# vLAR-group/OGC

Measured on AMD Instinct MI355X. Metric: point-clouds/sec (8192 pts) segnet fwd+bwd, higher is better.
Workload: dtype f32; 1 GPU; C4 KITTI-SF train_seg unsup: segnet_kitti fwd + OGC loss (dynamic+smooth+invariance) + bwd + Adam, 4 samples x 4 views x 8192 pts per GPU; n_point=8192, n_slot=10, parallelism=dp1, optimizer_stepped=True

## Files before the change

include/ogc_ops.h:

```cpp
#ifndef OGC_OPS_H
#define OGC_OPS_H

#ifdef __cplusplus
extern "C" {
#endif

typedef void *ogc_stream_t;
typedef unsigned short ogc_bf16_t;

enum {
    OGC_OK = 0,
    OGC_ERR_INVALID_ARG = -1,
    OGC_ERR_LAUNCH = -2,
    OGC_ERR_UNSUPPORTED = -3
};

#define OGC_VERSION 208
int ogc_version(void);
int ogc_distance_contracted(void);
int ogc_set_deterministic(int on);
int ogc_get_deterministic(void);
const char *ogc_last_error(void);

int ogc_furthest_point_sampling(int b, int n, int m, const float *xyz, float *temp,
// ... 150 lines not shown

int ogc_soft_carry(int b, int n1, int n2, int c, float temperature, const float *p1, const float *p2, const float *x,
                   float *out, ogc_stream_t stream);

#define OGC_SCAN_CROP_TILE 1024
#define OGC_SCAN_CROP_CAMERA_DOUBLES 36
int ogc_scan_crop_camera(int n, int stride, const float *scan, const double *cam, float clip_distance, float depth_thresh,
                         float *out_pc, int *keep_idx, int *count, ogc_stream_t stream);
int ogc_scan_crop_front(int n, int stride, const float *scan, float *out_pc, int *keep_idx, int *count, ogc_stream_t stream);
int ogc_scan_crop_tile(void);

#define OGC_BOX_SEGM_CHUNK 128
#define OGC_BOX_SEGM_BOX_DOUBLES 18
int ogc_box_segm(int n, int k, const float *pc, int sign_x, int sign_y, int sign_z, const double *boxes, const int *ids,
                 int *segm, int *semantic_segm, ogc_stream_t stream);
int ogc_box_segm_chunk(void);

int ogc_kittisf_unproject(int height, int width, const unsigned short *disp1, const unsigned short *disp2,
                          const unsigned short *flow, const unsigned short *inst, float fb, float f, float p02, float p03,
                          float p12, float p13, float p23, float depth_thresh, const int *select_semantics, int n_select,
                          float *pc1, float *pc2, int *segm, int *keep_idx, int *count, ogc_stream_t stream);

int ogc_png_unfilter(const unsigned char *in, unsigned char *out, int height, int row_bytes, int bpp);

int ogc_attention_fwd(int b, int lq, int lk, int h, int d, float scale, const float *q, int ldq, const float *k,
                      int ldk, const float *v, int ldv, float *out, float *prob, ogc_stream_t stream);
int ogc_attention_bwd(int b, int lq, int lk, int h, int d, float scale, const float *q, int ldq, const float *k,
                      int ldk, const float *v, int ldv, const float *out, const float *prob, const float *dout,
                      float *dq, int lddq, float *dk, int lddk, float *dv, int lddv, ogc_stream_t stream);

int ogc_small_linear_fwd(int rows, int n_in, int n_out, const float *x, const float *weight, const float *bias,
                         float *y, ogc_stream_t stream);
int ogc_small_linear_bwd(int rows, int n_in, int n_out, const float *x, const float *weight, const float *grad_y,
                         float *grad_x, float *grad_weight, float *grad_bias, ogc_stream_t stream);

int ogc_conv1x1_wgrad_moments(int b, int cin, int cout, int hw, int relu, const float *y_prev, const float *pa,
                              const float *pb, const float *grad_y, float *moments, ogc_stream_t stream);
int ogc_gn_moments_combine(int b, int cin, int cout, int hw, int groups, const float *moments, const float *w,
                           const float *pa, const float *pb, const float *mean, const float *rstd, const float *gamma,
                           float *grad_w, float *coef, float *grad_gamma, float *grad_beta, ogc_stream_t stream);
int ogc_conv1x1_dgrad_adjoint(int b, int cin, int cout, int hw, int relu, const float *w, const float *grad_y,
                              const float *y_prev, const float *pa, const float *pb, const float *coef, float *grad_prev,
                              ogc_stream_t stream);

int ogc_first_conv_stats(int b, int c1, int c0, int hw, int groups, const float *x0, const float *w1, double *stats,
                         ogc_stream_t stream);
int ogc_conv1x1_gemm_affine_first(int b, int M, int K, int hw, int relu, int groups, int c0, const float *w, const float *x0,
                                  const float *w1, const float *pa, const float *pb, float *out, double *stats,
                                  ogc_stream_t stream);
int ogc_conv1x1_wgrad_moments_first(int b, int cin, int cout, int hw, int relu, int c0, const float *x0, const float *w1,
                                    const float *pa, const float *pb, const float *grad_y, float *moments,
                                    ogc_stream_t stream);
int ogc_conv1x1_dgrad_adjoint_first(int b, int cin, int cout, int hw, int relu, int c0, const float *w, const float *grad_y,
                                    const float *x0, const float *w1, const float *pa, const float *pb, const float *coef,
                                    float *grad_w1, ogc_stream_t stream);

int ogc_group_norm_maxpool_bwd_sparse(int b, int c, int p, int s, int groups, int relu, const float *x,
                                      const float *x_at_argmax, const float *gamma, const float *mean, const float *rstd, const float *out, const int *argmax,
                                      const float *grad_out, float *coef2, float *inj, float *grad_gamma,
                                      float *grad_beta, double *ws, ogc_stream_t stream);
int ogc_conv1x1_wgrad_moments_pooled(int b, int cin, int cout, int hw, int relu, int nsample, const float *y_prev,
                                     const float *pa, const float *pb, const float *y, const float *coef2,
                                     const float *inj, float *moments, ogc_stream_t stream);
int ogc_conv1x1_dgrad_adjoint_pooled(int b, int cin, int cout, int hw, int relu, int nsample, const float *w, const float *y,
                                     const float *coef2, const float *inj, const float *y_prev, const float *pa,
                                     const float *pb, const float *coef, float *grad_prev, ogc_stream_t stream);

int ogc_live_steps(int b, int p, int nsample, const int *idx, int *live, int *n_live, ogc_stream_t stream);
int ogc_conv1x1_wgrad_moments_pooled_live(int b, int cin, int cout, int hw, int relu, int nsample, const float *y_prev,
                                          const float *pa, const float *pb, const float *y, const float *coef2,
                                          const float *inj, const int *live, const int *n_live, int live_cap, float *moments,
                                          ogc_stream_t stream);
int ogc_conv1x1_dgrad_adjoint_pooled_live(int b, int cin, int cout, int hw, int relu, int nsample, const float *w, const float *y,
                                          const float *coef2, const float *inj, const float *y_prev, const float *pa,
                                          const float *pb, const float *coef, const int *live, const int *n_live, int live_cap,
                                          float *grad_prev, ogc_stream_t stream);
int ogc_conv1x1_wgrad_moments_first_live(int b, int cin, int cout, int hw, int relu, int c0, int nsample, const float *x0,
                                         const float *w1, const float *pa, const float *pb, const float *grad_y,
                                         const int *live, const int *n_live, int live_cap, float *moments, ogc_stream_t stream);
int ogc_conv1x1_dgrad_adjoint_first_live(int b, int cin, int cout, int hw, int relu, int c0, int nsample, const float *w,
                                         const float *grad_y, const float *x0, const float *w1, const float *pa, const float *pb,
                                         const float *coef, const int *live, const int *n_live, int live_cap, float *grad_w1,
                                         ogc_stream_t stream);

int ogc_mlp_chain_pool_supported(int c0, int c1, int c2, int c3, int nsample);
int ogc_mlp_chain_pool(int b, int c0, int c1, int c2, int c3, int p, int nsample, const float *x, const float *wt1,
                       const float *b1, const float *wt2, const float *b2, const float *wt3, const float *b3, float *out,
                       ogc_stream_t stream);

int ogc_corr_layer_pool_supported(int cf, int c1, int c2, int c3, int nsample);
int ogc_corr_layer_pool(int b, int cf, int c1, int c2, int c3, int n1, int n2, int nsample, const float *pos1,
                        const float *pos2, const float *feat1, const float *feat2, const int *idx, const float *wt1,
                        const float *b1, const float *wt2, const float *b2, const float *wt3, const float *b3, float *out,
                        ogc_stream_t stream);

long long ogc_slot_masks_ws_floats(int b, int d, int n, int k);
int ogc_slot_masks_fwd(int b, int d, int n, int k, float temperature, const float *feats, const float *slots,
                       float *mask, ogc_stream_t stream);
int ogc_slot_masks_bwd(int b, int d, int n, int k, float temperature, const float *feats, const float *slots,
                       const float *mask, const float *grad_mask, float *grad_feats, float *grad_slots, float *ws,
                       ogc_stream_t stream);

int ogc_group_norm_stats_slots(void);
int ogc_group_norm_bwd_slots(void);
int ogc_group_norm_fwd(int b, int c, int hw, int groups, float eps, int relu, const float *x,
                       const float *gamma, const float *beta, float *y, float *mean, float *rstd,
                       double *ws, ogc_stream_t stream);
int ogc_group_norm_bwd(int b, int c, int hw, int groups, int relu, const float *x, const float *gamma,
                       const float *beta, const float *mean, const float *rstd, const float *grad_y,
                       float *grad_x, float *grad_gamma, float *grad_beta, double *ws, ogc_stream_t stream);

int ogc_group_norm_maxpool_fwd(int b, int c, int p, int s, int groups, float eps, int relu, const float *x,
                               const float *gamma, const float *beta, float *out, int *argmax, float *mean,
                               float *rstd, double *ws, ogc_stream_t stream);
int ogc_group_norm_maxpool_bwd(int b, int c, int p, int s, int groups, int relu, const float *x,
                               const float *gamma, const float *mean, const float *rstd, const float *out,
                               const int *argmax, const float *grad_out, float *grad_x, float *grad_gamma,
                               float *grad_beta, double *ws, ogc_stream_t stream);
int ogc_group_norm_maxpool_bwd_ext(int b, int c, int p, int s, int groups, int relu, const float *x,
                                   const float *x_at_argmax, const float *gamma, const float *mean, const float *rstd,
                                   const float *out, const int *argmax, const float *grad_out, float *grad_x,
                                   float *grad_gamma, float *grad_beta, double *ws, ogc_stream_t stream);

int ogc_batch_norm_fwd(int b, int c, int hw, float eps, int relu, int training, float momentum, const float *x,
                       const float *gamma, const float *beta, float *running_mean, float *running_var, float *y,
                       float *mean, float *rstd, double *ws, const double *stats, int slots, ogc_stream_t stream);
int ogc_batch_norm_bwd(int b, int c, int hw, int relu, int training, const float *x, const float *gamma,
                       const float *beta, const float *mean, const float *rstd, const float *grad_y, float *grad_x,
                       float *grad_gamma, float *grad_beta, double *ws, ogc_stream_t stream);
int ogc_batch_norm_maxpool_fwd(int b, int c, int p, int s, float eps, int relu, int training, float momentum,
                               const float *x, const float *gamma, const float *beta, float *running_mean,
                               float *running_var, float *out, int *argmax, float *mean, float *rstd, double *ws,
                               const double *stats, int slots, ogc_stream_t stream);
int ogc_batch_norm_maxpool_bwd(int b, int c, int p, int s, int relu, int training, const float *x, const float *gamma,
                               const float *mean, const float *rstd, const float *out, const int *argmax,
                               const float *grad_out, float *grad_x, float *grad_gamma, float *grad_beta, double *ws,
                               ogc_stream_t stream);

int ogc_conv1x1_wgrad(int b, int cin, int cout, int hw, const float *x, const float *dy, float *dw,
                      ogc_stream_t stream);

int ogc_conv1x1_gemm(int b, int M, int K, int hw, int transpose_a, const float *w, const float *in,
                     float *out, ogc_stream_t stream);

int ogc_conv1x1_gn_slots(void);
int ogc_conv1x1_gemm_stats_supported(int b, int M, int K, int hw, int affine);
int ogc_conv1x1_gemm_stream_supported(int b, int M, int K, int hw);
int ogc_conv1x1_gemm_any(int b, int M, int K, int hw, int transpose_a, const float *w, const float *in, float *out,
                         ogc_stream_t stream);

int ogc_set_matmul_precision(int bf16);
int ogc_conv1x1_gemm_gnstats(int b, int M, int K, int hw, int groups, const float *w, const float *in, float *out,
                             double *stats, ogc_stream_t stream);

int ogc_group_norm_coeffs(int b, int c, int hw, int groups, float eps, const float *x, const float *gamma,
                          const float *beta, const double *stats, int slots, double *ws, float *mean, float *rstd,
                          float *a, float *bb, ogc_stream_t stream);
int ogc_conv1x1_gemm_affine(int b, int M, int K, int hw, int relu, int groups, const float *w, const float *in,
                            const float *pa, const float *pb, float *out, double *stats, ogc_stream_t stream);
int ogc_conv1x1_wgrad_affine(int b, int cin, int cout, int hw, int relu, const float *x, const float *pa,
                             const float *pb, const float *dy, float *dw, ogc_stream_t stream);
int ogc_conv1x1_wgrad_affine_pooled(int b, int cin, int cout, int hw, int relu, int nsample, const float *x, const float *pa,
                                    const float *pb, const float *y, const float *coef2, const float *inj, float *dw,
                                    ogc_stream_t stream);
int ogc_conv1x1_dgrad_pooled(int b, int cin, int cout, int hw, int nsample, const float *w, const float *y, const float *coef2,
                             const float *inj, float *grad_z, ogc_stream_t stream);
// ... 87 lines not shown
```

ogc_amd/_lib.py:

```python
import ctypes
import os

_HERE = os.path.dirname(os.path.abspath(__file__))
FMAD = os.environ.get("OGC_FMAD", "0") == "1"
DETERMINISTIC = os.environ.get("OGC_DETERMINISTIC", "0") == "1"
LIB_PATH = os.path.join(_HERE, "csrc", "libogc_ops_fmad.so" if FMAD else "libogc_ops.so")

_vp = ctypes.c_void_p
_int = ctypes.c_int
_flt = ctypes.c_float
_dbl = ctypes.c_double
_ll = ctypes.c_longlong

SIGNATURES = {
    "ogc_set_deterministic": [_int],
    "ogc_group_linear_fwd_direct": [_int, _int, _int, _int, _int, _int, _int, _vp, _vp, _vp, _vp, _vp, _vp, _vp],
    "ogc_get_deterministic": [],
    "ogc_furthest_point_sampling": [_int, _int, _int, _vp, _vp, _vp, _vp],
    "ogc_furthest_point_sampling_chain": [_int, _int, _int, _vp, _vp, _vp, _vp, _vp, _vp],
    "ogc_gather_points": [_int, _int, _int, _int, _vp, _vp, _vp, _vp],
    "ogc_gather_points_grad": [_int, _int, _int, _int, _vp, _vp, _vp, _vp],
    "ogc_knn": [_int, _int, _int, _int, _vp, _vp, _vp, _vp, _vp],
    "ogc_three_nn": [_int, _int, _int, _vp, _vp, _vp, _vp, _vp],
    "ogc_three_interpolate": [_int, _int, _int, _int, _vp, _vp, _vp, _vp, _vp],
# ... 18 lines not shown
    "ogc_chamfer_terms": [_int, _int, _int, _int, _vp, _vp, _vp, _vp, _vp, _vp, _vp],
    "ogc_chamfer_terms_grad": [_int, _int, _int, _int, _vp, _vp, _vp, _vp, _vp, _vp, _vp, _vp],
    "ogc_gather_xyz_pair": [_int, _int, _int, _vp, _vp, _vp, _vp, _vp],
    "ogc_flow_advance": [_int, _int, _flt, _vp, _vp, _vp, _vp, _vp, _vp, _vp, _vp],
    "ogc_linear_cn": [_int, _int, _int, _int, _vp, _vp, _vp, _vp, _vp],
    "ogc_three_nn_weights": [_int, _int, _int, _vp, _vp, _vp],
    "ogc_soft_corr_flow": [_int, _int, _int, _int, _flt, _vp, _vp, _vp, _vp, _vp, _vp, _vp],
    "ogc_gru_reset": [_int, _int, _int, _int, _int, _vp, _ll, _vp, _vp, _vp],
    "ogc_gru_blend": [_int, _int, _int, _int, _vp, _ll, _vp, _ll, _vp, _ll, _vp, _vp],
    "ogc_zero_arena_begin": [_vp, _int, _vp],
    "ogc_zero_arena_end": [],
    "ogc_adam_max_tensors": [],
    "ogc_adam_chunk": [],
    "ogc_adam_step": [_int, _int, _vp, _vp, _vp, _vp, _vp, _dbl, _dbl, _dbl, _dbl, _dbl, _vp],
    "ogc_kabsch_rotation": [_int, _vp, _vp, _vp, _vp],
    "ogc_rigid_icp": [_int, _int, _vp, _vp, _vp, _int, _dbl, _vp, _vp, _vp, _vp],
    "ogc_ground_plane_fit": [_int, _int, _vp, _int, _int, _dbl, _dbl, _int, _vp, _vp, _vp, _vp],
    "ogc_seg_eval": [_int, _int, _int, _vp, _vp, _int, _vp, _vp, _vp, _vp, _vp, _vp, _vp, _vp, _vp, _vp, _vp],
    "ogc_seg_eval_ignore": [_int, _int, _int, _vp, _vp, _vp, _int, _vp, _vp, _vp, _vp, _vp, _vp, _vp, _vp, _vp, _vp, _vp, _vp],
    "ogc_flow_eval": [_int, _int, _vp, _vp, _dbl, _dbl, _vp, _vp, _vp],
    "ogc_lsap_maximize": [_int, _int, _vp, _vp, _vp],
    "ogc_sup_loss_ws_doubles": [_int, _int, _int],
    "ogc_sup_match_cost": [_int, _int, _int, _vp, _vp, _vp, _int, _dbl, _dbl, _vp, _vp, _vp, _vp],
    "ogc_sup_mask_loss_fwd": [_int, _int, _int, _vp, _vp, _vp, _vp, _int, _dbl, _dbl, _vp, _vp, _vp, _vp],
    "ogc_sup_mask_loss_bwd": [_int, _int, _int, _vp, _vp, _vp, _vp, _int, _dbl, _dbl, _vp, _dbl, _dbl, _vp, _vp, _vp],
    "ogc_rigid_moments": [_int, _int, _int, _vp, _vp, _vp, _vp, _vp, _vp, _vp],
    "ogc_rigid_translation": [_int, _vp, _vp, _vp, _vp, _vp],
    "ogc_rigid_blend": [_int, _int, _int, _int, _int, _vp, _vp, _vp, _vp, _vp, _vp, _vp, _vp],
    "ogc_mask_iou": [_int, _int, _int, _vp, _vp, _vp, _vp, _vp],
    "ogc_matched_distance": [_int, _int, _int, _int, _int, _vp, _vp, _vp, _vp, _vp, _vp, _vp, _vp, _vp],
    "ogc_soft_nn_target": [_int, _int, _int, _int, _flt, _vp, _vp, _vp, _vp, _vp, _vp],
    "ogc_soft_carry": [_int, _int, _int, _int, _flt, _vp, _vp, _vp, _vp, _vp],
    "ogc_scan_crop_camera": [_int, _int, _vp, _vp, _flt, _flt, _vp, _vp, _vp, _vp],
    "ogc_scan_crop_front": [_int, _int, _vp, _vp, _vp, _vp, _vp],
    "ogc_scan_crop_tile": [],
    "ogc_box_segm": [_int, _int, _vp, _int, _int, _int, _vp, _vp, _vp, _vp, _vp],
    "ogc_box_segm_chunk": [],
    "ogc_kittisf_unproject": [_int, _int, _vp, _vp, _vp, _vp, _flt, _flt, _flt, _flt, _flt, _flt, _flt, _flt, _vp, _int,
                              _vp, _vp, _vp, _vp, _vp, _vp],
    "ogc_png_unfilter": [_vp, _vp, _int, _int, _int],
    "ogc_group_concat": [_int, _int, _int, _int, _int, _vp, _vp, _vp, _vp, _vp, _vp],
    "ogc_group_linear_fwd": [_int, _int, _int, _int, _int, _int, _vp, _vp, _vp, _vp, _vp, _vp, _vp],
    "ogc_group_linear_bwd": [_int, _int, _int, _int, _int, _vp, _vp, _vp, _vp, _vp, _vp],
    "ogc_group_concat_grad": [_int, _int, _int, _int, _int, _vp, _vp, _vp, _vp],
    "ogc_neighbour_consistency_fwd": [_int, _int, _int, _int, _int, _vp, _vp, _vp, _vp],
    "ogc_reverse_neighbours": [_int, _int, _int, _vp, _vp, _vp, _vp, _vp, _vp],
    "ogc_neighbour_consistency_bwd": [_int, _int, _int, _int, _int, _vp, _vp, _vp, _vp, _vp, _vp, _vp, _vp],
    "ogc_sym_eigvals": [_int, _int, _vp, _vp, _vp],
    "ogc_group_norm_fwd": [_int, _int, _int, _int, _flt, _int, _vp, _vp, _vp, _vp, _vp, _vp, _vp, _vp],
    "ogc_group_norm_bwd": [_int, _int, _int, _int, _int, _vp, _vp, _vp, _vp, _vp, _vp, _vp, _vp, _vp, _vp, _vp],
    "ogc_group_norm_maxpool_fwd": [_int, _int, _int, _int, _int, _flt, _int, _vp, _vp, _vp, _vp, _vp, _vp, _vp, _vp, _vp],
    "ogc_conv1x1_gemm": [_int, _int, _int, _int, _int, _vp, _vp, _vp, _vp],
    "ogc_attention_fwd": [_int, _int, _int, _int, _int, _flt, _vp, _int, _vp, _int, _vp, _int, _vp, _vp, _vp],
    "ogc_attention_bwd": [_int, _int, _int, _int, _int, _flt, _vp, _int, _vp, _int, _vp, _int, _vp, _vp, _vp, _vp, _int,
                          _vp, _int, _vp, _int, _vp],
    "ogc_conv1x1_gemm_affine_pool": [_int, _int, _int, _int, _int, _int, _int, _vp, _vp, _vp, _vp, _vp, _vp, _vp, _vp, _vp,
                                     _vp],
    "ogc_group_norm_pool_extremes": [_int, _int, _int, _int, _int, _flt, _int, _vp, _vp, _vp, _vp, _vp, _vp, _vp, _vp, _vp,
                                     _int, _vp],
    "ogc_small_linear_fwd": [_int, _int, _int, _vp, _vp, _vp, _vp, _vp],
    "ogc_small_linear_bwd": [_int, _int, _int, _vp, _vp, _vp, _vp, _vp, _vp, _vp],
    "ogc_conv1x1_wgrad_moments": [_int, _int, _int, _int, _int, _vp, _vp, _vp, _vp, _vp, _vp],
    "ogc_gn_moments_combine": [_int, _int, _int, _int, _int, _vp, _vp, _vp, _vp, _vp, _vp, _vp, _vp, _vp, _vp, _vp, _vp],
    "ogc_conv1x1_dgrad_adjoint": [_int, _int, _int, _int, _int, _vp, _vp, _vp, _vp, _vp, _vp, _vp, _vp],
    "ogc_first_conv_stats": [_int, _int, _int, _int, _int, _vp, _vp, _vp, _vp],
    "ogc_conv1x1_gemm_affine_first": [_int, _int, _int, _int, _int, _int, _int, _vp, _vp, _vp, _vp, _vp, _vp, _vp, _vp],
    "ogc_conv1x1_wgrad_moments_first": [_int, _int, _int, _int, _int, _int, _vp, _vp, _vp, _vp, _vp, _vp, _vp],
    "ogc_conv1x1_dgrad_adjoint_first": [_int, _int, _int, _int, _int, _int, _vp, _vp, _vp, _vp, _vp, _vp, _vp, _vp, _vp],
    "ogc_group_norm_maxpool_bwd_sparse": [_int, _int, _int, _int, _int, _int, _vp, _vp, _vp, _vp, _vp, _vp, _vp, _vp, _vp, _vp,
                                          _vp, _vp, _vp, _vp],
    "ogc_group_norm_maxpool_bwd_ext": [_int, _int, _int, _int, _int, _int, _vp, _vp, _vp, _vp, _vp, _vp, _vp, _vp, _vp, _vp,
                                       _vp, _vp, _vp],
    "ogc_conv1x1_wgrad_moments_pooled": [_int, _int, _int, _int, _int, _int, _vp, _vp, _vp, _vp, _vp, _vp, _vp, _vp],
    "ogc_conv1x1_dgrad_adjoint_pooled": [_int, _int, _int, _int, _int, _int, _vp, _vp, _vp, _vp, _vp, _vp, _vp, _vp, _vp, _vp],
    "ogc_live_steps": [_int, _int, _int, _vp, _vp, _vp, _vp],
    "ogc_conv1x1_wgrad_moments_pooled_live": [_int, _int, _int, _int, _int, _int, _vp, _vp, _vp, _vp, _vp, _vp, _vp, _vp, _int, _vp,
                                              _vp],
    "ogc_conv1x1_dgrad_adjoint_pooled_live": [_int, _int, _int, _int, _int, _int, _vp, _vp, _vp, _vp, _vp, _vp, _vp, _vp, _vp, _vp,
                                              _int, _vp, _vp],
    "ogc_conv1x1_wgrad_moments_first_live": [_int, _int, _int, _int, _int, _int, _int, _vp, _vp, _vp, _vp, _vp, _vp, _vp, _int, _vp,
                                             _vp],
    "ogc_conv1x1_dgrad_adjoint_first_live": [_int, _int, _int, _int, _int, _int, _int, _vp, _vp, _vp, _vp, _vp, _vp, _vp, _vp, _vp,
                                             _int, _vp, _vp],
    "ogc_mlp_chain_pool_supported": [_int, _int, _int, _int, _int],
    "ogc_mlp_chain_pool":[_int, _int, _int, _int, _int, _int, _int, _vp, _vp, _vp, _vp, _vp, _vp, _vp, _vp, _vp],
    "ogc_corr_layer_pool_supported": [_int, _int, _int, _int, _int],
    "ogc_corr_layer_pool": [_int, _int, _int, _int, _int, _int, _int, _int, _vp, _vp, _vp, _vp, _vp, _vp, _vp, _vp, _vp, _vp,
                            _vp, _vp, _vp],
    "ogc_slot_masks_ws_floats": [_int, _int, _int, _int],
    "ogc_slot_masks_fwd": [_int, _int, _int, _int, _flt, _vp, _vp, _vp, _vp],
    "ogc_slot_masks_bwd": [_int, _int, _int, _int, _flt, _vp, _vp, _vp, _vp, _vp, _vp, _vp, _vp],
    "ogc_conv1x1_gn_slots": [],
    "ogc_conv1x1_gemm_stats_supported": [_int, _int, _int, _int, _int],
    "ogc_conv1x1_gemm_stream_supported": [_int, _int, _int, _int],
    "ogc_conv1x1_gemm_any": [_int, _int, _int, _int, _int, _vp, _vp, _vp, _vp],
    "ogc_set_matmul_precision": [_int],
    "ogc_group_norm_stats_slots": [],
    "ogc_group_norm_bwd_slots": [],
    "ogc_group_norm_coeffs": [_int, _int, _int, _int, _flt, _vp, _vp, _vp, _vp, _int, _vp, _vp, _vp, _vp, _vp, _vp],
    "ogc_conv1x1_gemm_affine": [_int, _int, _int, _int, _int, _int, _vp, _vp, _vp, _vp, _vp, _vp, _vp],
    "ogc_conv1x1_wgrad_affine": [_int, _int, _int, _int, _int, _vp, _vp, _vp, _vp, _vp, _vp],
    "ogc_conv1x1_wgrad_affine_pooled": [_int, _int, _int, _int, _int, _int, _vp, _vp, _vp, _vp, _vp, _vp, _vp, _vp],
    "ogc_conv1x1_dgrad_pooled": [_int, _int, _int, _int, _int, _vp, _vp, _vp, _vp, _vp, _vp],
    "ogc_batch_norm_fwd": [_int, _int, _int, _flt, _int, _int, _flt, _vp, _vp, _vp, _vp, _vp, _vp, _vp, _vp, _vp, _vp,
                           _int, _vp],
    "ogc_batch_norm_bwd": [_int, _int, _int, _int, _int, _vp, _vp, _vp, _vp, _vp, _vp, _vp, _vp, _vp, _vp, _vp],
    "ogc_batch_norm_maxpool_fwd": [_int, _int, _int, _int, _flt, _int, _int, _flt, _vp, _vp, _vp, _vp, _vp, _vp, _vp,
                                   _vp, _vp, _vp, _vp, _int, _vp],
    "ogc_batch_norm_maxpool_bwd": [_int, _int, _int, _int, _int, _int, _vp, _vp, _vp, _vp, _vp, _vp, _vp, _vp, _vp,
                                   _vp, _vp, _vp],
    "ogc_conv1x1_gemm_gnstats": [_int, _int, _int, _int, _int, _vp, _vp, _vp, _vp, _vp],
    "ogc_group_norm_fwd_stats": [_int, _int, _int, _int, _flt, _int, _vp, _vp, _vp, _vp, _vp, _vp, _vp, _int, _vp],
    "ogc_group_norm_maxpool_fwd_stats": [_int, _int, _int, _int, _int, _flt, _int, _vp, _vp, _vp, _vp, _vp, _vp, _vp,
                                         _vp, _int, _vp],
    "ogc_conv1x1_wgrad": [_int, _int, _int, _int, _vp, _vp, _vp, _vp],
    "ogc_group_norm_maxpool_bwd": [_int, _int, _int, _int, _int, _int, _vp, _vp, _vp, _vp, _vp, _vp, _vp, _vp, _vp, _vp,
                                   _vp, _vp],
}

for _n in ("ogc_group_linear_fwd", "ogc_group_points_grad_rev", "ogc_conv1x1_gemm", "ogc_conv1x1_gemm_affine",
           "ogc_conv1x1_gemm_affine_pool", "ogc_conv1x1_wgrad_affine", "ogc_conv1x1_wgrad_affine_pooled",
           "ogc_conv1x1_dgrad_pooled", "ogc_conv1x1_wgrad_moments", "ogc_conv1x1_wgrad_moments_pooled",
           "ogc_conv1x1_dgrad_adjoint", "ogc_conv1x1_dgrad_adjoint_pooled", "ogc_group_norm_bwd",
           "ogc_group_norm_maxpool_bwd_sparse", "ogc_group_points_grad_rev_dwx"):
    SIGNATURES[_n + "_h"] = SIGNATURES[_n]
SIGNATURES["ogc_group_linear_fwd_direct_h"] = SIGNATURES["ogc_group_linear_fwd_direct"]
SIGNATURES["ogc_conv1x1_wgrad_xf_h"] = SIGNATURES["ogc_conv1x1_wgrad"]
SIGNATURES["ogc_group_linear_fwd_pt_h"] = SIGNATURES["ogc_group_linear_fwd"]

HEADER_VERSION = 208
_lib = None
_fns = {}


class OgcOpsError(RuntimeError):
    pass


def load():
    global _lib
    if _lib is None:
        if not os.path.exists(LIB_PATH):
            raise OgcOpsError(
                "libogc_ops.so not found at %s — build it with `python ogc_amd/csrc/build.py` "
                "(there is no CPU fallback)" % LIB_PATH)
        L = ctypes.CDLL(LIB_PATH)
        for name, argtypes in SIGNATURES.items():
            fn = getattr(L, name)
            fn.argtypes = argtypes
            fn.restype = _int
        L.ogc_version.restype = _int
        if L.ogc_version() != HEADER_VERSION:
            raise OgcOpsError("libogc_ops.so at %s is version %d, this package binds version %d of include/ogc_ops.h — rebuild it "
                              "with `python ogc_amd/csrc/build.py --force`" % (LIB_PATH, L.ogc_version(), HEADER_VERSION))
        L.ogc_distance_contracted.restype = _int
        if bool(L.ogc_distance_contracted()) != FMAD:
            raise OgcOpsError("%s evaluates distances %s, OGC_FMAD asked for the other form" %
                              (LIB_PATH, "contracted (fma)" if L.ogc_distance_contracted() else "un-contracted"))
        L.ogc_slot_masks_ws_floats.restype = ctypes.c_longlong
        L.ogc_cell_grid_bytes.restype = ctypes.c_longlong
        L.ogc_sup_loss_ws_doubles.restype = ctypes.c_longlong
        L.ogc_last_error.restype = ctypes.c_char_p
        L.ogc_set_deterministic(1 if DETERMINISTIC else 0)
        _lib = L
    return _lib

# ... 61 lines not shown
```

ogc_amd/csrc/build.py:

```python
import os
import subprocess
import sys
from concurrent.futures import ThreadPoolExecutor

HERE = os.path.dirname(os.path.abspath(__file__))
SOURCES = ["api.hip", "det.hip", "knn.hip", "ball_query.hip", "fps.hip", "gather_group.hip", "interpolate.hip", "kabsch.hip", "rigid_icp.hip", "ground_plane.hip", "seg_eval.hip", "flow_eval.hip", "sup_loss.hip", "small_solvers.hip", "neighbour_loss.hip", "soft_nn.hip", "soft_carry.hip", "scan_prepare.hip", "kittisf_prepare.hip", "seg_loss.hip", "group_norm.hip", "batch_norm.hip", "grid.hip", "grid_ball_query.hip", "grid_knn.hip", "conv1x1.hip", "conv1x1_h.hip", "conv1x1_wgrad.hip", "attention.hip", "slot_masks.hip", "small_linear.hip", "loss_glue.hip", "mlp_chain.hip", "gn_fused_bwd.hip", "adam.hip", "gemm_chunk.hip", "chamfer.hip", "flow_step.hip"]
HEADERS = ["ogc_common.h", "grid.h", "grid_dev.h", "conv_stage.h", "conv1x1_shared.h", "act_io.h", "norm_dev.h", "conv1x1_epilogue.h", "first_conv.h", "wgrad_tile_body.inc", "wgrad_shared_body.inc", "svd3.h", "png_unfilter.h", os.path.join("..", "..", "include", "ogc_ops.h")]
LIB = os.path.join(HERE, "libogc_ops.so")
FMAD_SOURCES = ["knn.hip", "ball_query.hip", "fps.hip", "grid.hip", "grid_ball_query.hip", "grid_knn.hip"]
LIB_FMAD = os.path.join(HERE, "libogc_ops_fmad.so")
HIPCC = os.environ.get("HIPCC", "/opt/rocm/bin/hipcc")
FLAGS = [
    "--offload-arch=gfx950", "-O3", "-std=c++17", "-fPIC",
    "-ffp-contract=off",
    "-munsafe-fp-atomics",
    "-mllvm", "-amdgpu-mfma-vgpr-form=1",
    "-Wall", "-Wno-unused-function",
]


def _newer(target, deps):
    if not os.path.exists(target):
        return True
    t = os.path.getmtime(target)
    return any(os.path.getmtime(d) > t for d in deps)


def build(force=False, verbose=False):
    hdrs = [os.path.join(HERE, h) for h in HEADERS] + [os.path.abspath(__file__)]
    objs, objs_fmad, jobs = [], [], []
    for s in SOURCES:
        src = os.path.join(HERE, s)
        obj = os.path.join(HERE, s.replace(".hip", ".o"))
        objs.append(obj)
        if force or _newer(obj, [src] + hdrs):
            jobs.append([HIPCC] + FLAGS + ["-c", src, "-o", obj])
        if s in FMAD_SOURCES:
            obj_f = os.path.join(HERE, s.replace(".hip", ".fmad.o"))
            objs_fmad.append(obj_f)
            if force or _newer(obj_f, [src] + hdrs):
                jobs.append([HIPCC] + FLAGS + ["-DOGC_FMAD=1", "-c", src, "-o", obj_f])
        else:
            objs_fmad.append(obj)

    def run(cmd):
        if verbose:
            print(" ".join(cmd), flush=True)
        subprocess.check_call(cmd)

    with ThreadPoolExecutor(max_workers=min(8, max(1, len(jobs)))) as ex:
        list(ex.map(run, jobs))
    if force or jobs or _newer(LIB, objs):
        run([HIPCC, "--offload-arch=gfx950", "-shared", "-fPIC", "-o", LIB] + objs)
    if force or jobs or _newer(LIB_FMAD, objs_fmad):
        run([HIPCC, "--offload-arch=gfx950", "-shared", "-fPIC", "-o", LIB_FMAD] + objs_fmad)
    return LIB


if __name__ == "__main__":
    print(build(force="--force" in sys.argv, verbose="--verbose" in sys.argv))
```

ogc_amd/csrc/conv1x1.hip:

```cpp
#include "conv1x1_shared.h"
#include "act_io.h"
#include "conv1x1_epilogue.h"
#include "first_conv.h"

int ogc_g_matmul_bf16 = 0;


namespace {


template <bool TRANSPOSE_A, int KQ, bool STATS, bool PRO, bool BF, bool POOL = false, typename IT = float, typename OT = float,
          int FIRST = 0>
__global__ __launch_bounds__(WG_WAVES *OGC_WAVE) void conv1x1_gemm_kernel(int M, int K, int hw, int groups,
                                                                          const float *__restrict__ w,
                                                                          const IT *__restrict__ in,
                                                                          OT *__restrict__ out,
                                                                          double *__restrict__ stats,
                                                                          const float *__restrict__ pa,
                                                                          const float *__restrict__ pb, int pro_relu,
                                                                          PoolOut pool = PoolOut(), FirstIn first = FirstIn()) {
    extern __shared__ __attribute__((aligned(16))) float a_lds[];
    __shared__ __attribute__((aligned(16))) float s_w1[FIRST ? FC_MAX_ROWS * FC_MAX_C0 : 4];
    __shared__ double s_stats[STATS ? 64 : 1];
    __shared__ __attribute__((aligned(16))) float s_sign[POOL ? 64 : 4];
    const int lane = threadIdx.x & 63, wave = threadIdx.x >> 6;
    const int j = lane & 15, kk = lane >> 4;
    const int b = blockIdx.y;
    const int p0 = (blockIdx.x * WG_WAVES + wave) * 64;
    const int Kq = (K + 3) >> 2, a_ld = ogc_a_ld(Kq);
    const bool live = p0 < hw;
    const IT *inb = in + (size_t)b * K * hw;
    OT *outb = out + (size_t)b * M * hw;
    if (STATS && threadIdx.x < 2 * groups) s_stats[threadIdx.x] = 0.0;

    float4 xin[KQ];
    if constexpr (FIRST > 0) {
        static_assert(KQ * 4 <= FC_MAX_ROWS && sizeof(IT) == 4 && !TRANSPOSE_A, "first-layer form: fp32, at most 64 rows of W1");
        ogc_first_stage_w1<WG_WAVES * OGC_WAVE>(s_w1, first.w1, K, first.c0);
        float4 x0v[FIRST];
        ogc_first_load_raw<FIRST>(x0v, first.x0 + (size_t)b * first.c0 * hw + (live ? p0 + 4 * j : 0), first.c0, hw);
        ogc_first_mask<FIRST>(x0v, first.c0, live);
        __syncthreads();
#pragma unroll
        for (int q = 0; q < KQ; ++q) {
            float w1r[FIRST];
            ogc_first_w1_row<FIRST>(w1r, s_w1, q * 4 + kk);
            xin[q] = ogc_first_row<FIRST>(x0v, w1r);
        }
    } else {
#pragma unroll
    for (int q = 0; q < KQ; ++q) {
        const int row = q * 4 + kk;
        xin[q] = (live && q < Kq && row < K) ? ogc_ld4(inb + (size_t)row * hw + p0 + 4 * j) : make_float4(0.f, 0.f, 0.f, 0.f);
    }
    }
    if (PRO) {
        constexpr int CH = 8;
#pragma unroll
        for (int q0 = 0; q0 < KQ; q0 += CH) {
            float ca[CH], cb[CH];
#pragma unroll
            for (int u = 0; u < CH; ++u) {
                const int q = q0 + u, row = q * 4 + kk;
                const bool have = q < KQ && live && q < Kq && row < K;
                ca[u] = have ? pa[(size_t)b * K + row] : 0.f;
                cb[u] = have ? pb[(size_t)b * K + row] : 0.f;
            }
#pragma unroll
            for (int u = 0; u < CH; ++u) {
                const int q = q0 + u;
                if (q < KQ) {
                    float4 v = xin[q];
                    v.x = fmaf(ca[u], v.x, cb[u]); v.y = fmaf(ca[u], v.y, cb[u]);
                    v.z = fmaf(ca[u], v.z, cb[u]); v.w = fmaf(ca[u], v.w, cb[u]);
                    if (pro_relu) { v.x = fmaxf(v.x, 0.f); v.y = fmaxf(v.y, 0.f); v.z = fmaxf(v.z, 0.f); v.w = fmaxf(v.w, 0.f); }
                    xin[q] = v;
                }
            }
        }
    }
    constexpr int GQ = (KQ + 3) / 4;
    v4s xb[BF ? GQ : 1][4];
    if constexpr (BF) {
#pragma unroll
        for (int g = 0; g < GQ; ++g) {
            float4 r[4];
#pragma unroll
            for (int i = 0; i < 4; ++i) r[i] = 4 * g + i < KQ ? xin[4 * g + i] : make_float4(0.f, 0.f, 0.f, 0.f);
            xb[g][0] = ogc_pack_bf16(r[0].x, r[1].x, r[2].x, r[3].x);
            xb[g][1] = ogc_pack_bf16(r[0].y, r[1].y, r[2].y, r[3].y);
            xb[g][2] = ogc_pack_bf16(r[0].z, r[1].z, r[2].z, r[3].z);
            xb[g][3] = ogc_pack_bf16(r[0].w, r[1].w, r[2].w, r[3].w);
        }
    }
    const int cpg = STATS ? M / groups : 1;
    for (int m0 = 0; m0 < M; m0 += 64) {
        __syncthreads();
        if constexpr (BF) {
            v4s *a_bf = reinterpret_cast<v4s *>(a_lds);
            const int Gq = (Kq + 3) >> 2;
            for (int t = threadIdx.x; t < Gq * 256; t += WG_WAVES * OGC_WAVE) {
                const int kr = t & 3, mi = (t >> 2) & 63, g = t >> 8;
                const int m = m0 + mi;
                float v[4];
#pragma unroll
                for (int i = 0; i < 4; ++i) {
                    const int k = 4 * (4 * g + i) + kr;
                    v[i] = (m < M && k < K) ? (TRANSPOSE_A ? w[(size_t)k * M + m] : w[(size_t)m * K + k]) : 0.f;
                }
                a_bf[t] = ogc_pack_bf16(v[0], v[1], v[2], v[3]);
            }
        } else {
        ogc_stage_weight_tile<TRANSPOSE_A, WG_WAVES>(a_lds, w, m0, M, K, Kq);
        }
        if constexpr (POOL) {
            if (threadIdx.x < 64) s_sign[threadIdx.x] = (m0 + (int)threadIdx.x < M && pool.sign[m0 + threadIdx.x] < 0.f) ? -1.f : 1.f;
        }
        __syncthreads();
        const int nblk = min(4, (M - m0 + 15) >> 4);
        v4f acc[4][4];
#pragma unroll
        for (int a = 0; a < 4; ++a)
#pragma unroll
            for (int c = 0; c < 4; ++c) acc[a][c] = (v4f){0.f, 0.f, 0.f, 0.f};
        if constexpr (BF) {
            const v4s *a_bf = reinterpret_cast<const v4s *>(a_lds);
#pragma unroll
            for (int g = 0; g + 1 < GQ; g += 2) {
                if (4 * (g + 1) < Kq) {
                    v4s av0[4], av1[4];
#pragma unroll
                    for (int a = 0; a < 4; ++a) {
                        av0[a] = a_bf[(g * 64 + a * 16 + j) * 4 + kk];
                        av1[a] = a_bf[((g + 1) * 64 + a * 16 + j) * 4 + kk];
                    }
#pragma unroll
                    for (int a = 0; a < 4; ++a) {
                        if (a < nblk) {
#pragma unroll
                            for (int c = 0; c < 4; ++c)
                                acc[a][c] = ogc_mfma_bf16_k32(av0[a], av1[a], xb[g][c], xb[g + 1][c], acc[a][c]);
                        }
                    }
                } else if (4 * g < Kq) {
                    v4s av[4];
#pragma unroll
                    for (int a = 0; a < 4; ++a) av[a] = a_bf[(g * 64 + a * 16 + j) * 4 + kk];
#pragma unroll
                    for (int a = 0; a < 4; ++a) {
                        if (a < nblk) {
#pragma unroll
                            for (int c = 0; c < 4; ++c)
                                acc[a][c] = __builtin_amdgcn_mfma_f32_16x16x16bf16_1k(av[a], xb[g][c], acc[a][c], 0, 0, 0);
                        }
                    }
                }
            }
            if constexpr (GQ % 2 == 1) {
                constexpr int g = GQ - 1;
                if (4 * g < Kq) {
                    v4s av[4];
#pragma unroll
                    for (int a = 0; a < 4; ++a) av[a] = a_bf[(g * 64 + a * 16 + j) * 4 + kk];
#pragma unroll
                    for (int a = 0; a < 4; ++a) {
                        if (a < nblk) {
#pragma unroll
                            for (int c = 0; c < 4; ++c)
                                acc[a][c] = __builtin_amdgcn_mfma_f32_16x16x16bf16_1k(av[a], xb[g][c], acc[a][c], 0, 0, 0);
                        }
                    }
                }
            }
        } else {
#pragma unroll
        for (int q = 0; q < KQ; ++q) {
            if (q < Kq) {
                float av[4];
#pragma unroll
                for (int a = 0; a < 4; ++a) av[a] = a_lds[(a * 16 + j) * a_ld + q * 4 + kk];
#pragma unroll
                for (int a = 0; a < 4; ++a) {
                    if (a < nblk) {
                        acc[a][0] = __builtin_amdgcn_mfma_f32_16x16x4f32(av[a], xin[q].x, acc[a][0], 0, 0, 0);
                        acc[a][1] = __builtin_amdgcn_mfma_f32_16x16x4f32(av[a], xin[q].y, acc[a][1], 0, 0, 0);
                        acc[a][2] = __builtin_amdgcn_mfma_f32_16x16x4f32(av[a], xin[q].z, acc[a][2], 0, 0, 0);
                        acc[a][3] = __builtin_amdgcn_mfma_f32_16x16x4f32(av[a], xin[q].w, acc[a][3], 0, 0, 0);
                    }
                }
            }
        }
        }
        if (live) {
            if constexpr (sizeof(OT) == 2 && (STATS || POOL)) {
#pragma unroll
                for (int a = 0; a < 4; ++a)
#pragma unroll
                    for (int c = 0; c < 4; ++c)
#pragma unroll
                        for (int r = 0; r < 4; ++r) acc[a][c][r] = ogc_as_stored<OT>(acc[a][c][r]);
            }
#pragma unroll
            for (int a = 0; a < 4; ++a)
#pragma unroll
                for (int r = 0; r < 4; ++r) {
                    const int m = m0 + a * 16 + kk * 4 + r;
                    if (m < M) {
                        const float4 o = make_float4(acc[a][0][r], acc[a][1][r], acc[a][2][r], acc[a][3][r]);
                        ogc_st4(outb + (size_t)m * hw + p0 + 4 * j, o);
                    }
                }
            if constexpr (POOL) {
                const int centres = hw / pool.s;
                const int centre = (p0 + 4 * j) / pool.s;
                const size_t o0 = ((size_t)b * M + m0 + kk * 4) * centres + centre;
                if (pool.s == 64) ogc_pool_extremes_epilogue<16>(acc, nblk, s_sign, j, kk, m0, M, centres, 64, pool.yext + o0, pool.aext + o0);
                else if (pool.s == 32) ogc_pool_extremes_epilogue<8>(acc, nblk, s_sign, j, kk, m0, M, centres, 32, pool.yext + o0, pool.aext + o0);
                else ogc_pool_extremes_epilogue<4>(acc, nblk, s_sign, j, kk, m0, M, centres, 16, pool.yext + o0, pool.aext + o0);
            }
            if (STATS) {
#pragma unroll
                for (int a = 0; a < 4; ++a) {
                    if (a < nblk) {
                        float sm = 0.f, sq = 0.f;
#pragma unroll
                        for (int r = 0; r < 4; ++r)
#pragma unroll
                            for (int c = 0; c < 4; ++c) {
                                const float v = acc[a][c][r];
                                sm += v;
                                sq += v * v;
                            }
                        sm += ogc_dpp_f32<0xB1>(sm); sq += ogc_dpp_f32<0xB1>(sq);
                        sm += ogc_dpp_f32<0x4E>(sm); sq += ogc_dpp_f32<0x4E>(sq);
                        sm += ogc_dpp_f32<0x141>(sm); sq += ogc_dpp_f32<0x141>(sq);
                        sm += ogc_dpp_f32<0x140>(sm); sq += ogc_dpp_f32<0x140>(sq);
                        const int m = m0 + a * 16 + kk * 4;
                        if (j == 0 && m < M) {
                            const int g = m / cpg;
                            atomicAdd(&s_stats[2 * g], (double)sm);
                            atomicAdd(&s_stats[2 * g + 1], (double)sq);
                        }
                    }
                }
            }
        }
    }
    if (STATS) {
        __syncthreads();
        if (threadIdx.x < 2 * groups) {
            const int slot = blockIdx.x % GN_SLOTS;
            double *dst = stats + ((size_t)slot * gridDim.y + b) * 2 * groups;
            atomicAdd(dst + threadIdx.x, s_stats[threadIdx.x]);
        }
    }
}

template <int KQ, bool PRO, bool EXACT, bool STATS = false, bool POOL = false, bool DUAL = false, bool TRANS = false>
__global__ __launch_bounds__(WG_WAVES *OGC_WAVE, DUAL ? 2 : 1) void conv1x1_gemm_stream_kernel(int M, int K, int hw, int ntiles,
                                                                                 const float *__restrict__ w,
                                                                                 const float *__restrict__ in,
                                                                                 float *__restrict__ out,
                                                                                 const float *__restrict__ pa,
                                                                                 const float *__restrict__ pb, int pro_relu,
                                                                                 int groups = 1, int nbatch = 1,
                                                                                 double *__restrict__ stats = nullptr,
                                                                                 PoolOut pool = PoolOut()) {
    extern __shared__ __attribute__((aligned(16))) float a_lds[];
    const int lane = threadIdx.x & 63, wave = __builtin_amdgcn_readfirstlane(threadIdx.x >> 6);
    const int j = lane & 15, kk = lane >> 4;
    const int Kq = (K + 3) >> 2, Mt = (M + 63) >> 6, a_ld = ogc_a_ld(Kq);
    const int tiles_per_img = hw >> 6;
    for (int mt = 0; mt < Mt; ++mt)
        ogc_stage_weight_tile<TRANS, WG_WAVES>(a_lds + (size_t)mt * 64 * a_ld, w, mt * 64, M, K, Kq);
    float *sgn_all = a_lds + (size_t)Mt * 64 * a_ld + (PRO ? WG_WAVES * 2 * FW_KQ_MAX * 4 : 0) + WG_WAVES * 4 * 16 * 2 * 2;
    if constexpr (POOL) {
        for (int t = threadIdx.x; t < Mt * 64; t += WG_WAVES * OGC_WAVE) sgn_all[t] = (t < M && pool.sign[t] < 0.f) ? -1.f : 1.f;
    }
    __syncthreads();
    const int nw = gridDim.x * WG_WAVES;
    const unsigned off_main = (unsigned)(kk * hw + 4 * j);
    const unsigned off_last = (unsigned)(min(kk, K - 1 - (Kq - 1) * 4) * hw + 4 * j);
    auto load_tile = [&](int t, float4(&x)[KQ]) {
        t = min(t, ntiles - 1);
        const int b = t / tiles_per_img, p0 = (t - b * tiles_per_img) * 64;
        const float *inb = in + (size_t)b * K * hw + p0;
#pragma unroll
        for (int q = 0; q < KQ; ++q)
            if (EXACT || q < Kq) {
                const float *rowq = inb + (size_t)(q * 4) * hw;
                x[q] = *reinterpret_cast<const float4 *>(rowq + ((EXACT ? q == KQ - 1 : q == Kq - 1) ? off_last : off_main));
            }
    };
    float *cw = a_lds + (size_t)Mt * 64 * a_ld + wave * (2 * KQ * 4);
    int coef_b = -1;
    double *sacc = reinterpret_cast<double *>(a_lds + (size_t)Mt * 64 * a_ld + (PRO ? WG_WAVES * 2 * FW_KQ_MAX * 4 : 0)) +
                   wave * (4 * 16 * 2);
    int stat_b = -1;
    auto flush_stats = [&]() {
        if constexpr (STATS) {
            if (stat_b >= 0) {
                const int cpg = M / groups;
                double *dst = stats + ((size_t)(blockIdx.x % GN_SLOTS) * nbatch + stat_b) * 2 * groups;
                if (lane < Mt * 16) {
                    const int m = (lane >> 4) * 64 + ((lane >> 2) & 3) * 16 + (lane & 3) * 4;
                    if (m < M) {
                        unsafeAtomicAdd(dst + 2 * (m / cpg), sacc[2 * lane]);
                        unsafeAtomicAdd(dst + 2 * (m / cpg) + 1, sacc[2 * lane + 1]);
                    }
                }
            }
            if (lane < 64) { sacc[2 * lane] = 0.0; sacc[2 * lane + 1] = 0.0; }
            __builtin_amdgcn_wave_barrier();
        }
    };
    auto compute_store = [&](int t, float4(&x)[KQ]) {
        const int b = t / tiles_per_img, p0 = (t - b * tiles_per_img) * 64;
        if constexpr (STATS) {
            if (b != stat_b) { flush_stats(); stat_b = b; }
// ... 412 lines not shown
        for (int a = 0; a < 4; ++a) {
            if (a < nblk) {
                float sm = 0.f, sq = 0.f;
#pragma unroll
                for (int r = 0; r < 4; ++r) {
                    float w[CP];
                    ogc_first_w1_row<CP>(w, s_w1, a * 16 + kk * 4 + r);
                    const float4 v = ogc_first_row<CP>(x, w);
                    sm += v.x; sq += v.x * v.x;
                    sm += v.y; sq += v.y * v.y;
                    sm += v.z; sq += v.z * v.z;
                    sm += v.w; sq += v.w * v.w;
                }
                sm += ogc_dpp_f32<0xB1>(sm); sq += ogc_dpp_f32<0xB1>(sq);
                sm += ogc_dpp_f32<0x4E>(sm); sq += ogc_dpp_f32<0x4E>(sq);
                sm += ogc_dpp_f32<0x141>(sm); sq += ogc_dpp_f32<0x141>(sq);
                sm += ogc_dpp_f32<0x140>(sm); sq += ogc_dpp_f32<0x140>(sq);
                dsm[a] += (double)sm;
                dsq[a] += (double)sq;
            }
        }
    }
    const int cpg = c1 / groups;
#pragma unroll
    for (int a = 0; a < 4; ++a) {
        const int m = a * 16 + kk * 4;
        if (j == 0 && m < c1) {
            atomicAdd(&s_stats[2 * (m / cpg)], dsm[a]);
            atomicAdd(&s_stats[2 * (m / cpg) + 1], dsq[a]);
        }
    }
    __syncthreads();
    if (threadIdx.x < 2 * groups) {
        double *dst = stats + ((size_t)(blockIdx.x % GN_SLOTS) * gridDim.y + b) * 2 * groups;
        atomicAdd(dst + threadIdx.x, s_stats[threadIdx.x]);
    }
}

int first_check(const char *name, int b, int c1, int c0, int hw, const float *x0, const float *w1) {
    OGC_REQUIRE(b >= 0 && c1 >= 1 && c0 >= 1 && hw >= 1, "%s: bad shape", name);
    OGC_REQUIRE(x0 && w1, "%s: null pointer", name);
    if (c0 > FC_MAX_C0 || c1 > FC_MAX_ROWS || (hw & 63) != 0 || ((uintptr_t)x0 & 15) != 0) {
        ogc_set_error("%s: needs c0 <= %d, c1 <= %d, hw %% 64 == 0 and a 16-byte aligned x0 (c0=%d, c1=%d, hw=%d)", name, FC_MAX_C0,
                      FC_MAX_ROWS, c0, c1, hw);
        return OGC_ERR_UNSUPPORTED;
    }
    OGC_REQUIRE((long long)FC_MAX_ROWS * hw < (1ll << 31) && b <= 32768, "%s: one sample exceeds 32-bit indexing", name);
    return OGC_OK;
}

}

int ogc_first_check(const char *name, int b, int c1, int c0, int hw, const float *x0, const float *w1) {
    return first_check(name, b, c1, c0, hw, x0, w1);
}

extern "C" int ogc_first_conv_stats(int b, int c1, int c0, int hw, int groups, const float *x0, const float *w1, double *stats,
                                    ogc_stream_t stream) {
    const int rc = first_check("ogc_first_conv_stats", b, c1, c0, hw, x0, w1);
    if (rc != OGC_OK) return rc;
    OGC_REQUIRE(stats, "ogc_first_conv_stats: null pointer");
    if (groups < 1 || groups > 32 || c1 % groups != 0 || (c1 / groups) % 4 != 0) {
        ogc_set_error("ogc_first_conv_stats: needs 1 <= groups <= 32 and (c1 / groups) %% 4 == 0 (c1=%d, groups=%d)", c1, groups);
        return OGC_ERR_UNSUPPORTED;
    }
    if (b == 0) return OGC_OK;
    hipStream_t s = (hipStream_t)stream;
    if (ogc_zero_async(stats, sizeof(double) * 2 * GN_SLOTS * (size_t)b * groups, s) != hipSuccess) {
        ogc_set_error("ogc_first_conv_stats: memset failed");
        return OGC_ERR_LAUNCH;
    }
    const int tiles = ogc_divup(hw, 64 * WG_WAVES);
    int run = ogc_divup((long long)tiles * b, 2048);
    if (run > 8) run = 8;
    dim3 grid(ogc_divup(tiles, run), b), block(WG_WAVES * OGC_WAVE);
    const int cp = ogc_first_cp(c0);
    if (cp == 3) hipLaunchKernelGGL(first_conv_stats_kernel<3>, grid, block, 0, s, c1, c0, hw, groups, run, x0, w1, stats);
    else if (cp == 6) hipLaunchKernelGGL(first_conv_stats_kernel<6>, grid, block, 0, s, c1, c0, hw, groups, run, x0, w1, stats);
    else hipLaunchKernelGGL(first_conv_stats_kernel<8>, grid, block, 0, s, c1, c0, hw, groups, run, x0, w1, stats);
    OGC_CHECK_LAUNCH("ogc_first_conv_stats");
    return OGC_OK;
}

extern "C" int ogc_conv1x1_gemm_affine_first(int b, int M, int K, int hw, int relu, int groups, int c0, const float *w,
                                             const float *x0, const float *w1, const float *pa, const float *pb, float *out,
                                             double *stats, ogc_stream_t stream) {
    const char *name = "ogc_conv1x1_gemm_affine_first";
    int rc = first_check(name, b, K, c0, hw, x0, w1);
    if (rc != OGC_OK) return rc;
    OGC_REQUIRE(M >= 1 && w && pa && pb && out && stats, "%s: bad shape or null pointer", name);
    if (groups < 1 || groups > 32 || M % groups != 0 || (M / groups) % 4 != 0 || ((uintptr_t)out & 15) != 0 || g_matmul_bf16) {
        ogc_set_error("%s: needs fp32 operands, 1 <= groups <= 32, (M / groups) %% 4 == 0 and a 16-byte aligned output (M=%d, "
                      "groups=%d)", name, M, groups);
        return OGC_ERR_UNSUPPORTED;
    }
    OGC_REQUIRE((long long)M * hw < (1ll << 31) && b <= 65535, "%s: one sample exceeds 32-bit indexing", name);
    if (b == 0) return OGC_OK;
    hipStream_t s = (hipStream_t)stream;
    if (ogc_zero_async(stats, sizeof(double) * 2 * GN_SLOTS * (size_t)b * groups, s) != hipSuccess) {
        ogc_set_error("%s: memset failed", name);
        return OGC_ERR_LAUNCH;
    }
    const int Kq = (K + 3) / 4, cp = ogc_first_cp(c0);
    const size_t lds = (size_t)64 * ogc_a_ld(Kq) * sizeof(float);
    dim3 grid(ogc_divup(hw, 64 * WG_WAVES), b);
    FirstIn first;
    first.x0 = x0; first.w1 = w1; first.c0 = c0;
#define OGC_GEMM_FIRST(KQV, CPV)                                                                                           \
    hipLaunchKernelGGL((conv1x1_gemm_kernel<false, KQV, true, true, false, false, float, float, CPV>), grid,               \
                       dim3(WG_WAVES * OGC_WAVE), lds, s, M, K, hw, groups, w, (const float *)nullptr, out, stats, pa, pb, relu, \
                       PoolOut(), first)
    if (Kq <= 8) {
        if (cp == 3) OGC_GEMM_FIRST(8, 3); else if (cp == 6) OGC_GEMM_FIRST(8, 6); else OGC_GEMM_FIRST(8, 8);
    } else {
        if (cp == 3) OGC_GEMM_FIRST(16, 3); else if (cp == 6) OGC_GEMM_FIRST(16, 6); else OGC_GEMM_FIRST(16, 8);
    }
#undef OGC_GEMM_FIRST
    OGC_CHECK_LAUNCH(name);
    return OGC_OK;
}
```

ogc_amd/csrc/conv1x1_epilogue.h:

```cpp
#pragma once
#include "conv1x1_shared.h"

namespace {

constexpr int FW_KQ_MAX = 40;
constexpr int GN_SLOTS = 16;

template <int CTRL>
__device__ __forceinline__ float ogc_max_dpp_f32(float x) {
    float r;
    if constexpr (CTRL == 0xB1)
        asm("s_nop 1\n\tv_max_f32_dpp %0, %1, %1 quad_perm:[1,0,3,2] row_mask:0xf bank_mask:0xf" : "=v"(r) : "v"(x));
    else if constexpr (CTRL == 0x4E)
        asm("s_nop 1\n\tv_max_f32_dpp %0, %1, %1 quad_perm:[2,3,0,1] row_mask:0xf bank_mask:0xf" : "=v"(r) : "v"(x));
    else if constexpr (CTRL == 0x141)
        asm("s_nop 1\n\tv_max_f32_dpp %0, %1, %1 row_half_mirror row_mask:0xf bank_mask:0xf" : "=v"(r) : "v"(x));
    else
        asm("s_nop 1\n\tv_max_f32_dpp %0, %1, %1 row_mirror row_mask:0xf bank_mask:0xf" : "=v"(r) : "v"(x));
    return r;
}
__device__ __forceinline__ float ogc_max3_f32(float a, float b, float c) {
    float r;
    asm("v_max3_f32 %0, %1, %2, %3" : "=v"(r) : "v"(a), "v"(b), "v"(c));
    return r;
}
__device__ __forceinline__ float ogc_max2_f32(float a, float b) {
    float r;
    asm("v_max_f32 %0, %1, %2" : "=v"(r) : "v"(a), "v"(b));
    return r;
}

struct PoolOut {
    float *yext;
    int *aext;
    const float *sign;
    int s;
};

template <int SEG, typename ACC>
__device__ __forceinline__ void ogc_pool_extremes_epilogue(const ACC (&acc)[4][4], int nblk, const float *sgn, int j, int kk,
                                                           int m0, int M, int centres, int pool_s, float *ye, int *ae) {
    const bool writer = (j & (SEG - 1)) == 0;
#pragma unroll
    for (int a = 0; a < 4; ++a) {
        if (a < nblk) {
            const float4 sg4 = *reinterpret_cast<const float4 *>(sgn + a * 16 + kk * 4);
            const float sga[4] = {sg4.x, sg4.y, sg4.z, sg4.w};
#pragma unroll
            for (int r = 0; r < 4; ++r) {
                const int m = m0 + a * 16 + kk * 4 + r;
                const float sg = sga[r];
                const float v0 = sg * acc[a][0][r], v1 = sg * acc[a][1][r];
                const float v2 = sg * acc[a][2][r], v3 = sg * acc[a][3][r];
                float hi = ogc_max3_f32(v0, v1, ogc_max2_f32(v2, v3));
                hi = ogc_max_dpp_f32<0xB1>(hi);
                hi = ogc_max_dpp_f32<0x4E>(hi);
                if (SEG >= 8) hi = ogc_max_dpp_f32<0x141>(hi);
                if (SEG >= 16) hi = ogc_max_dpp_f32<0x140>(hi);
                unsigned idx = v3 == hi ? 4u * j + 3u : 64u;
                idx = v2 == hi ? 4u * j + 2u : idx;
                idx = v1 == hi ? 4u * j + 1u : idx;
                idx = v0 == hi ? 4u * j : idx;
                idx = min(idx, ogc_dpp_u32<0xB1>(idx));
                idx = min(idx, ogc_dpp_u32<0x4E>(idx));
                if (SEG >= 8) idx = min(idx, ogc_dpp_u32<0x141>(idx));
                if (SEG >= 16) idx = min(idx, ogc_dpp_u32<0x140>(idx));
                if (writer && m < M) {
                    const int o = (a * 16 + r) * centres;
                    ye[o] = sg * hi;
                    ae[o] = (int)(idx & (unsigned)(pool_s - 1));
                }
            }
        }
    }
}

template <auto KERNEL, typename... ARGS>
bool ogc_persistent_launch(size_t lds, int lds_cap, int per_cu, long long ntiles, hipStream_t s, ARGS... args) {
    static bool raised = false;
    if (!raised) {
        if (hipFuncSetAttribute(reinterpret_cast<const void *>(KERNEL), hipFuncAttributeMaxDynamicSharedMemorySize, lds_cap) != hipSuccess) {
            (void)hipGetLastError();
            return false;
        }
        raised = true;
    }
    long long wgs = 256ll * per_cu;
    if (wgs > ntiles / WG_WAVES) wgs = ntiles / WG_WAVES;
    hipLaunchKernelGGL(KERNEL, dim3((unsigned)wgs), dim3(WG_WAVES * OGC_WAVE), lds, s, args...);
    return true;
}

}
```

ogc_amd/csrc/gn_fused_bwd.hip:

```cpp
#include "conv1x1_shared.h"
#include "act_io.h"
#include "first_conv.h"

namespace {

constexpr int LIVE_SHIFT = 28;
constexpr int LIVE_MASK = (1 << LIVE_SHIFT) - 1;
struct LiveIn {
    const int *steps = nullptr;
    const int *n = nullptr;
    int cap = 0;
};

constexpr int LIVE_MAX_P = 32768;
__global__ __launch_bounds__(1024) void live_steps_kernel(int p, int s, const int *__restrict__ idx, int *__restrict__ steps,
                                                          int *__restrict__ n_live) {
    __shared__ int part[1024];
    __shared__ unsigned char cnt[LIVE_MAX_P];
    const int t = threadIdx.x, b = blockIdx.x, T = s >> 4;
    const int lane = t & 63, wave = t >> 6;
    const int *ib = idx + (size_t)b * p * s;
    int *out = steps + (size_t)b * p * T;
    const int row0 = lane & ~(s - 1);
    const unsigned long long row_mask = (s == 64 ? ~0ull : (1ull << s) - 1ull) << row0;
    const int total = p * s;
    for (int e0 = wave * 64; e0 < total; e0 += 1024) {
        const bool in = e0 + lane < total;
        const int v = in ? ib[e0 + lane] : 0;
        const int first = __shfl(v, row0);
        const unsigned long long differs = __builtin_amdgcn_ballot_w64(in && v != first) & row_mask;
        const int hi = differs ? 63 - __clzll(differs) - row0 : 0;
        if (in && lane == row0) cnt[(e0 + lane) / s] = (unsigned char)(min((hi + 1) >> 4, T - 1) + 1);
    }
    __syncthreads();
    const int per = (p + 1023) / 1024;
    const int c0 = min(t * per, p), c1 = min(c0 + per, p);
    int sum = 0;
    for (int c = c0; c < c1; ++c) sum += cnt[c];
    part[t] = sum;
    __syncthreads();
    for (int off = 1; off < 1024; off <<= 1) {
        const int v = t >= off ? part[t - off] : 0;
        __syncthreads();
        part[t] += v;
        __syncthreads();
    }
    int at = t > 0 ? part[t - 1] : 0;
    for (int c = c0; c < c1; ++c) {
        const int sl = cnt[c] - 1;
        for (int st = 0; st <= sl; ++st) out[at++] = (c * T + st) | (st == sl ? (T - 1 - sl) << LIVE_SHIFT : 0);
    }
    if (t == 1023) n_live[b] = part[1023];
}

template <int COB, int CIB, bool POOLED, typename AT = float, int FIRST = 0, bool LIST = false>
__global__ __launch_bounds__(WG_WAVES *OGC_WAVE) void wgrad_moments_kernel(int cin, int cout, int hw, int chunks,
                                                                           int steps_per_wave, int relu,
                                                                           const AT *__restrict__ x,
                                                                           const AT *__restrict__ dy,
                                                                           const float *__restrict__ aff_a,
                                                                           const float *__restrict__ aff_b,
                                                                           const float2 *__restrict__ coef2,
                                                                           const float2 *__restrict__ inj,
                                                                           int s_shift,
                                                                           float *__restrict__ hm,
                                                                           FirstIn first = FirstIn(), LiveIn ls = LiveIn()) {
    constexpr int XN = FIRST ? FIRST : CIB;
    __shared__ float red[WG_WAVES][COB * CIB * 256];
    const int lane = threadIdx.x & 63, wave = __builtin_amdgcn_readfirstlane(threadIdx.x >> 6);
    const int i = lane & 15, k = lane >> 4;
    const int img = blockIdx.x / chunks, chunk = blockIdx.x - img * chunks;
    const int co0 = blockIdx.y * (16 * COB), ci0 = blockIdx.z * (16 * CIB);
    int steps_per_img = hw >> 4;
    const int *lv_ = nullptr;
    if constexpr (LIST) {
        steps_per_img = min(ls.n[img], ls.cap);
        lv_ = ls.steps + (size_t)img * ls.cap;
        const int waves = chunks * WG_WAVES;
        steps_per_wave = ((steps_per_img + waves - 1) / waves + 1) & ~1;
        if (chunk * WG_WAVES * steps_per_wave >= steps_per_img) return;
    }
    const int first_step = (chunk * WG_WAVES + wave) * steps_per_wave;
    const int mine = max(0, min(steps_per_wave, steps_per_img - first_step));

    v4f acc1[COB][CIB], acc2[COB][CIB];
#pragma unroll
    for (int a = 0; a < COB; ++a)
#pragma unroll
        for (int c = 0; c < CIB; ++c) {
            acc1[a][c] = (v4f){0.f, 0.f, 0.f, 0.f};
            acc2[a][c] = (v4f){0.f, 0.f, 0.f, 0.f};
        }
    int yrow[COB], xrow[XN], jrow[COB];
    float ca[CIB], cb[CIB], pc2[COB], pc3[COB];
    float w1r[FIRST ? CIB : 1][FIRST ? FIRST : 1];
    const int centres = hw >> s_shift, smask = (1 << s_shift) - 1;
#pragma unroll
    for (int a = 0; a < COB; ++a) {
        const int row = min(co0 + a * 16 + i, cout - 1);
        yrow[a] = row * hw;
        if (POOLED) {
            const float2 cc = coef2[(size_t)img * cout + row];
            pc2[a] = cc.x;
            pc3[a] = cc.y;
            jrow[a] = row * centres;
        }
    }
    const float2 *jb_ = POOLED ? inj + (size_t)img * cout * centres : nullptr;
#pragma unroll
    for (int c = 0; c < CIB; ++c) {
        const int ch = min(ci0 + c * 16 + i, cin - 1);
        if constexpr (FIRST == 0) xrow[c] = ch * hw;
        ca[c] = aff_a[(size_t)img * cin + ch];
        cb[c] = aff_b[(size_t)img * cin + ch];
        if constexpr (FIRST > 0) {
#pragma unroll
            for (int e = 0; e < FIRST; ++e) w1r[c][e] = e < first.c0 ? first.w1[ch * first.c0 + min(e, first.c0 - 1)] : 0.f;
        }
    }
    if constexpr (FIRST > 0) {
#pragma unroll
        for (int e = 0; e < FIRST; ++e) xrow[e] = min(e, first.c0 - 1) * hw;
    }
    const AT *yb_ = dy + (size_t)img * cout * hw + 4 * k;
    const AT *xb_ = FIRST ? reinterpret_cast<const AT *>(first.x0) + (size_t)img * first.c0 * hw + 4 * k
                          : x + (size_t)img * cin * hw + 4 * k;
    int cur = min(first_step, steps_per_img - 1);
    const int stop = min(first_step + mine, steps_per_img) - 1;
    int ent = LIST ? lv_[cur] : 0;
    auto load = [&](float4(&yv)[COB], float4(&xv)[XN], float2(&jv)[COB], int &jpos, int &went) {
        const int pb = LIST ? min(ent & LIVE_MASK, (hw >> 4) - 1) * 16 : cur * 16;
        if constexpr (LIST) went = ent;
#pragma unroll
        for (int a = 0; a < COB; ++a) yv[a] = ogc_ld4(yb_ + yrow[a] + pb);
#pragma unroll
// ... 496 lines not shown
                    for (int g = 0; g + 1 < GQ; g += 2) {
                        if (4 * (g + 1) < Kq) {
                            const v4s av0 = a_bf[(g * 64 + a * 16 + j) * 4 + kk], av1 = a_bf[((g + 1) * 64 + a * 16 + j) * 4 + kk];
#pragma unroll
                            for (int c = 0; c < 4; ++c) acc[c] = ogc_mfma_bf16_k32(av0, av1, xb[g][c], xb[g + 1][c], acc[c]);
                        } else if (4 * g < Kq) {
                            const v4s av = a_bf[(g * 64 + a * 16 + j) * 4 + kk];
#pragma unroll
                            for (int c = 0; c < 4; ++c) acc[c] = __builtin_amdgcn_mfma_f32_16x16x16bf16_1k(av, xb[g][c], acc[c], 0, 0, 0);
                        }
                    }
                    if constexpr (GQ % 2 == 1) {
                        constexpr int g = GQ - 1;
                        if (4 * g < Kq) {
                            const v4s av = a_bf[(g * 64 + a * 16 + j) * 4 + kk];
#pragma unroll
                            for (int c = 0; c < 4; ++c) acc[c] = __builtin_amdgcn_mfma_f32_16x16x16bf16_1k(av, xb[g][c], acc[c], 0, 0, 0);
                        }
                    }
                } else {
#pragma unroll
                for (int q = 0; q < KQ; ++q) {
                    if (q < Kq) {
                        const float av = a_lds[(a * 16 + j) * a_ld + q * 4 + kk];
                        acc[0] = __builtin_amdgcn_mfma_f32_16x16x4f32(av, xin[q].x, acc[0], 0, 0, 0);
                        acc[1] = __builtin_amdgcn_mfma_f32_16x16x4f32(av, xin[q].y, acc[1], 0, 0, 0);
                        acc[2] = __builtin_amdgcn_mfma_f32_16x16x4f32(av, xin[q].z, acc[2], 0, 0, 0);
                        acc[3] = __builtin_amdgcn_mfma_f32_16x16x4f32(av, xin[q].w, acc[3], 0, 0, 0);
                    }
                }
                }
                if (live) {
#pragma unroll
                    for (int r = 0; r < 4; ++r) {
                        const int mi = a * 16 + kk * 4 + r, m = m0 + mi;
                        if (m < M) {
                            const float fa = cf[mi * 5], fb = cf[mi * 5 + 1], al = cf[mi * 5 + 2], c2 = cf[mi * 5 + 3], c3 = cf[mi * 5 + 4];
                            const float4 y = yv[r];
                            float4 g = make_float4(acc[0][r], acc[1][r], acc[2][r], acc[3][r]);
                            if (relu) {
                                g.x = fmaf(fa, y.x, fb) > 0.f ? g.x : 0.f; g.y = fmaf(fa, y.y, fb) > 0.f ? g.y : 0.f;
                                g.z = fmaf(fa, y.z, fb) > 0.f ? g.z : 0.f; g.w = fmaf(fa, y.w, fb) > 0.f ? g.w : 0.f;
                            }
                            float4 o;
                            o.x = fmaf(al, g.x, fmaf(c2, y.x, c3)); o.y = fmaf(al, g.y, fmaf(c2, y.y, c3));
                            o.z = fmaf(al, g.z, fmaf(c2, y.z, c3)); o.w = fmaf(al, g.w, fmaf(c2, y.w, c3));
                            if constexpr (FIRST > 0) {
                                float mine = 0.f;
                                if constexpr (LIST) o.w *= wl;
#pragma unroll
                                for (int c = 0; c < FIRST; ++c) {
                                    float d = fmaf(o.w, x0v[c].w, fmaf(o.z, x0v[c].z, fmaf(o.y, x0v[c].y, o.x * x0v[c].x)));
                                    d += ogc_dpp_f32<0xB1>(d);
                                    d += ogc_dpp_f32<0x4E>(d);
                                    d += ogc_dpp_f32<0x141>(d);
                                    d += ogc_dpp_f32<0x140>(d);
                                    mine = j == c ? d : mine;
                                }
                                if (j < first.c0) atomicAdd(&s_dw[m * FC_MAX_C0 + j], mine);
                            } else {
                                if (mine_ok) ogc_st4(outb + (size_t)m * hw + pos, o);
                            }
                        }
                    }
                }
            }
        }
    }
    }
    if constexpr (FIRST > 0) {
        __syncthreads();
        for (int t = threadIdx.x; t < M * first.c0; t += WG_WAVES * OGC_WAVE) {
            const float v = s_dw[(t / first.c0) * FC_MAX_C0 + t % first.c0];
            if (v != 0.0f) unsafeAtomicAdd(first.dw1 + t, v);
        }
    }
}

}

namespace {
int nsample_shift(int nsample) { return nsample == 16 ? 4 : nsample == 32 ? 5 : nsample == 64 ? 6 : -1; }

int live_check(const char *name, const int *live, const int *n_live, int live_cap, int hw, int nsample, LiveIn &ls) {
    OGC_REQUIRE(live && n_live, "%s: null live-step list", name);
    if (nsample != 32 && nsample != 64) {
        ogc_set_error("%s: the list form needs nsample 32 or 64 (nsample=%d)", name, nsample);
        return OGC_ERR_UNSUPPORTED;
    }
    OGC_REQUIRE(hw >= 16 && hw % nsample == 0 && (hw >> 4) <= LIVE_MASK && live_cap >= (hw >> 4),
                "%s: the live-step list holds %d entries per sample, hw=%d needs room for %d", name, live_cap, hw, hw >> 4);
    ls.steps = live; ls.n = n_live; ls.cap = live_cap;
    return OGC_OK;
}

template <typename AT>
int wgrad_moments_impl(const char *name, int b, int cin, int cout, int hw, int relu, const AT *y_prev, const float *pa,
                       const float *pb, const AT *grad_y, const float *coef2, const float *inj, int s_shift,
                       float *moments, ogc_stream_t stream, LiveIn ls = LiveIn()) {
    OGC_REQUIRE(b >= 0 && cin >= 1 && cout >= 1 && hw >= 1, "%s: bad shape", name);
    OGC_REQUIRE(y_prev && pa && pb && grad_y && moments, "%s: null pointer", name);
    if ((hw & (sizeof(AT) == 2 ? 31 : 15)) != 0 || (((uintptr_t)y_prev | (uintptr_t)grad_y) & 15) != 0) {
        ogc_set_error("%s: hw=%d must be a multiple of 16 (32 for 16-bit tensors) and the tensors 16-byte aligned", name, hw);
        return OGC_ERR_UNSUPPORTED;
    }
    if (sizeof(AT) == 2 && !ogc_g_matmul_bf16) {
        ogc_set_error("%s: 16-bit activations need ogc_set_matmul_precision(1)", name);
        return OGC_ERR_UNSUPPORTED;
    }
    OGC_REQUIRE((long long)cin * hw < (1ll << 31) && (long long)cout * hw < (1ll << 31) && b <= 32768,
                "%s: one sample exceeds 32-bit indexing", name);
    hipStream_t s = (hipStream_t)stream;
    if (b == 0) return OGC_OK;
    if (ogc_zero_async(moments, sizeof(float) * 2 * (size_t)b * cin * cout, s) != hipSuccess) {
        ogc_set_error("%s: memset failed", name);
        return OGC_ERR_LAUNCH;
    }
#define OGC_ML(A, C) moments_launch<A, C, AT>(b, cin, cout, hw, relu, y_prev, grad_y, pa, pb, coef2, inj, s_shift, moments, s, FirstIn(), ls)
    if (cout <= 16 && cin <= 16) OGC_ML(1, 1);
    else if (cout <= 32 && cin <= 16) OGC_ML(2, 1);
    else if (cout <= 32 && cin <= 32) OGC_ML(2, 2);
    else if (cin <= 16) OGC_ML(4, 1);
    else if (cin <= 32) OGC_ML(4, 2);
    else if (cout <= 32) OGC_ML(2, 4);
    else if (inj && sizeof(AT) == 4) OGC_ML(4, 2);
    else OGC_ML(4, 4);
#undef OGC_ML
    OGC_CHECK_LAUNCH(name);
    return OGC_OK;
}
}

extern "C" int ogc_conv1x1_wgrad_moments(int b, int cin, int cout, int hw, int relu, const float *y_prev, const float *pa,
                                         const float *pb, const float *grad_y, float *moments, ogc_stream_t stream) {
    return wgrad_moments_impl<float>("ogc_conv1x1_wgrad_moments", b, cin, cout, hw, relu, y_prev, pa, pb, grad_y, nullptr, nullptr, 0,
                                     moments, stream);
}

extern "C" int ogc_conv1x1_wgrad_moments_h(int b, int cin, int cout, int hw, int relu, const ogc_bf16_t *y_prev, const float *pa,
                                           const float *pb, const ogc_bf16_t *grad_y, float *moments, ogc_stream_t stream) {
    return wgrad_moments_impl<ogc_bf16>("ogc_conv1x1_wgrad_moments_h", b, cin, cout, hw, relu, y_prev, pa, pb, grad_y, nullptr,
                                        nullptr, 0, moments, stream);
}

namespace {
template <typename AT>
int wgrad_moments_pooled_impl(const char *name, int b, int cin, int cout, int hw, int relu, int nsample, const AT *y_prev,
                              const float *pa, const float *pb, const AT *y, const float *coef2, const float *inj,
                              float *moments, ogc_stream_t stream, LiveIn ls = LiveIn()) {
    const int sh = nsample_shift(nsample);
    if (sh < 0 || hw % nsample != 0 || (((uintptr_t)coef2 | (uintptr_t)inj) & 7) != 0) {
        ogc_set_error("%s: nsample=%d must be 16, 32 or 64 and divide hw=%d", name, nsample, hw);
        return OGC_ERR_UNSUPPORTED;
    }
    OGC_REQUIRE(b == 0 || (coef2 && inj), "%s: null pointer", name);
    return wgrad_moments_impl<AT>(name, b, cin, cout, hw, relu, y_prev, pa, pb, y, coef2, inj, sh, moments, stream, ls);
}
}

extern "C" int ogc_conv1x1_wgrad_moments_pooled(int b, int cin, int cout, int hw, int relu, int nsample, const float *y_prev,
                                                const float *pa, const float *pb, const float *y, const float *coef2,
                                                const float *inj, float *moments, ogc_stream_t stream) {
    return wgrad_moments_pooled_impl<float>("ogc_conv1x1_wgrad_moments_pooled", b, cin, cout, hw, relu, nsample, y_prev, pa, pb, y,
                                            coef2, inj, moments, stream);
}

extern "C" int ogc_conv1x1_wgrad_moments_pooled_live(int b, int cin, int cout, int hw, int relu, int nsample, const float *y_prev,
                                                     const float *pa, const float *pb, const float *y, const float *coef2,
                                                     const float *inj, const int *live, const int *n_live, int live_cap,
                                                     float *moments, ogc_stream_t stream) {
    const char *name = "ogc_conv1x1_wgrad_moments_pooled_live";
    LiveIn ls;
    const int rc = live_check(name, live, n_live, live_cap, hw, nsample, ls);
    if (rc != OGC_OK) return rc;
    return wgrad_moments_pooled_impl<float>(name, b, cin, cout, hw, relu, nsample, y_prev, pa, pb, y, coef2, inj, moments, stream, ls);
}

extern "C" int ogc_conv1x1_wgrad_moments_pooled_h(int b, int cin, int cout, int hw, int relu, int nsample,
// ... 197 lines not shown
    }
    if (b == 0) return OGC_OK;
    const int M = cin, K = cout, Kq = (K + 3) / 4;
    const size_t lds = ((size_t)64 * ogc_a_ld(Kq) + 64 * 5) * sizeof(float);
    const int tiles = ogc_divup(hw, 64 * WG_WAVES);
    int chunks = 768 / b;
    if (chunks < 1) chunks = 1;
    if (chunks > tiles) chunks = tiles;
    FirstIn first;
    first.x0 = x0; first.w1 = w1; first.c0 = c0; first.dw1 = grad_w1;
    first.run = ogc_divup(tiles, chunks);
    dim3 grid(ogc_divup(tiles, first.run), b);
    const int cp = ogc_first_cp(c0);
#define OGC_DGAF(KQV, CPV)                                                                                                  \
    do {                                                                                                                    \
        if (ls.steps)                                                                                                       \
            hipLaunchKernelGGL((dgrad_adjoint_kernel<KQV, false, float, false, CPV, true>), grid, dim3(WG_WAVES * OGC_WAVE), lds, s, M, \
                               K, hw, relu, w, grad_y, (const float *)nullptr, pa, pb, coef, (const float2 *)nullptr,       \
                               (const float2 *)nullptr, 0, (float *)nullptr, first, ls);                                    \
        else                                                                                                                \
            hipLaunchKernelGGL((dgrad_adjoint_kernel<KQV, false, float, false, CPV>), grid, dim3(WG_WAVES * OGC_WAVE), lds, s, M, K, \
                               hw, relu, w, grad_y, (const float *)nullptr, pa, pb, coef, (const float2 *)nullptr,          \
                               (const float2 *)nullptr, 0, (float *)nullptr, first, ls);                                    \
    } while (0)
    if (Kq <= 8) {
        if (cp == 3) OGC_DGAF(8, 3); else if (cp == 6) OGC_DGAF(8, 6); else OGC_DGAF(8, 8);
    } else {
        if (cp == 3) OGC_DGAF(16, 3); else if (cp == 6) OGC_DGAF(16, 6); else OGC_DGAF(16, 8);
    }
#undef OGC_DGAF
    OGC_CHECK_LAUNCH(name);
    return OGC_OK;
}
}

extern "C" int ogc_conv1x1_wgrad_moments_first(int b, int cin, int cout, int hw, int relu, int c0, const float *x0, const float *w1,
                                               const float *pa, const float *pb, const float *grad_y, float *moments,
                                               ogc_stream_t stream) {
    return wgrad_moments_first_impl("ogc_conv1x1_wgrad_moments_first", b, cin, cout, hw, relu, c0, x0, w1, pa, pb, grad_y, moments,
                                    stream);
}

extern "C" int ogc_conv1x1_dgrad_adjoint_first(int b, int cin, int cout, int hw, int relu, int c0, const float *w,
                                               const float *grad_y, const float *x0, const float *w1, const float *pa,
                                               const float *pb, const float *coef, float *grad_w1, ogc_stream_t stream) {
    return dgrad_adjoint_first_impl("ogc_conv1x1_dgrad_adjoint_first", b, cin, cout, hw, relu, c0, w, grad_y, x0, w1, pa, pb, coef,
                                    grad_w1, stream);
}

extern "C" int ogc_conv1x1_wgrad_moments_first_live(int b, int cin, int cout, int hw, int relu, int c0, int nsample, const float *x0,
                                                    const float *w1, const float *pa, const float *pb, const float *grad_y,
                                                    const int *live, const int *n_live, int live_cap, float *moments,
                                                    ogc_stream_t stream) {
    const char *name = "ogc_conv1x1_wgrad_moments_first_live";
    LiveIn ls;
    const int rc = live_check(name, live, n_live, live_cap, hw, nsample, ls);
    if (rc != OGC_OK) return rc;
    return wgrad_moments_first_impl(name, b, cin, cout, hw, relu, c0, x0, w1, pa, pb, grad_y, moments, stream, ls);
}

extern "C" int ogc_conv1x1_dgrad_adjoint_first_live(int b, int cin, int cout, int hw, int relu, int c0, int nsample, const float *w,
                                                    const float *grad_y, const float *x0, const float *w1, const float *pa,
                                                    const float *pb, const float *coef, const int *live, const int *n_live,
                                                    int live_cap, float *grad_w1, ogc_stream_t stream) {
    const char *name = "ogc_conv1x1_dgrad_adjoint_first_live";
    LiveIn ls;
    const int rc = live_check(name, live, n_live, live_cap, hw, nsample, ls);
    if (rc != OGC_OK) return rc;
    return dgrad_adjoint_first_impl(name, b, cin, cout, hw, relu, c0, w, grad_y, x0, w1, pa, pb, coef, grad_w1, stream, ls);
}

extern "C" int ogc_live_steps(int b, int p, int s, const int *idx, int *live, int *n_live, ogc_stream_t stream) {
    OGC_REQUIRE(b >= 0 && p >= 1, "ogc_live_steps: bad shape");
    if (s != 16 && s != 32 && s != 64) {
        ogc_set_error("ogc_live_steps: nsample=%d must be 16, 32 or 64", s);
        return OGC_ERR_UNSUPPORTED;
    }
    OGC_REQUIRE(idx && live && n_live, "ogc_live_steps: null pointer");
    if (p > LIVE_MAX_P) {
        ogc_set_error("ogc_live_steps: p=%d centres per sample, at most %d", p, LIVE_MAX_P);
        return OGC_ERR_UNSUPPORTED;
    }
    if (b == 0) return OGC_OK;
    hipLaunchKernelGGL(live_steps_kernel, dim3(b), dim3(1024), 0, (hipStream_t)stream, p, s, idx, live, n_live);
    OGC_CHECK_LAUNCH("ogc_live_steps");
    return OGC_OK;
}
```

ogc_amd/fused.py:

```python
import weakref

import torch
import torch.nn.functional as F
from torch.autograd import Function

from .pointnet2 import pointnet2 as _api



import collections as _collections
import functools as _functools

from .utils.zero_arena import zeroed_empty

GATE_MISSES = _collections.Counter()


def deterministic():
    from . import _lib
    return _lib.DETERMINISTIC

ACT16 = __import__("os").environ.get("OGC_ACT16", "1") != "0"


# ... 567 lines not shown
def rigid_residual_available(mask, loss_norm):
    return (mask.is_cuda and mask.dtype == torch.float32 and loss_norm in (1, 2) and mask.shape[-1] <= 32
            and getattr(_api._native, "rigid_blend_wrapper", None) is not None)


def rigid_residual(pc, pc2, mask, loss_norm):
    nat = _api._native
    pc, pc2, mask = pc.contiguous(), pc2.contiguous(), mask.contiguous()
    VB, N, K = mask.shape
    dev = mask.device
    with torch.no_grad():
        mom = zeroed_empty(VB * K * 16, torch.float64, dev)
        S = torch.empty(VB * K, 3, 3, dtype=torch.float32, device=dev)
        means = torch.empty(VB * K, 6, dtype=torch.float32, device=dev)
        nat.rigid_moments_wrapper(VB, N, K, pc, pc2, mask.detach(), mom, S, means)
        R = torch.empty_like(S)
        valid = torch.empty(VB * K, dtype=torch.int32, device=dev)
        nat.kabsch_rotation_wrapper(VB * K, S, R, valid)
        t = torch.empty(VB * K, 3, dtype=torch.float32, device=dev)
        nat.rigid_translation_wrapper(VB * K, means, valid, R, t)
    return _RigidBlend.apply(pc, pc2, mask, R, t, int(loss_norm))


class _MatchedDistance(Function):

    @staticmethod
    def forward(ctx, mask1, mask2, col12, col21, p):
        nat = _api._native
        PB, N, K = mask1.shape
        d12 = torch.empty(PB, N, dtype=torch.float32, device=mask1.device)
        d21 = torch.empty_like(d12)
        nat.matched_distance_wrapper(PB, N, K, p, 0, mask1, mask2, col12, col21, None, None, d12, d21)
        ctx.save_for_backward(mask1, mask2, col12, col21)
        ctx.p = p
        return d12, d21

    @staticmethod
    def backward(ctx, g12, g21):
        nat = _api._native
        mask1, mask2, col12, col21 = ctx.saved_tensors
        PB, N, K = mask1.shape
        gm1, gm2 = torch.empty_like(mask1), torch.empty_like(mask2)
        nat.matched_distance_wrapper(PB, N, K, ctx.p, 1, mask1, mask2, col12, col21, g12.contiguous(), g21.contiguous(),
                                     gm1, gm2)
        return gm1, gm2, None, None, None


@_gate
def matched_distance_available(mask, loss_norm, cross_entropy):
    return (mask.is_cuda and mask.dtype == torch.float32 and not cross_entropy and loss_norm in (1, 2)
            and mask.shape[-1] <= 32 and getattr(_api._native, "matched_distance_wrapper", None) is not None
            and getattr(_api._native, "lsap_maximize_wrapper", None) is not None)


def matched_distances(mask1, mask2, loss_norm):
    nat = _api._native
    mask1, mask2 = mask1.contiguous(), mask2.contiguous()
    PB, N, K = mask1.shape
    dev = mask1.device
    with torch.no_grad():
        counts = zeroed_empty(PB * K * K, torch.int32, dev)
        iou = torch.empty(PB, K, K, dtype=torch.float32, device=dev)
        nat.mask_iou_wrapper(PB, N, K, mask1.detach(), mask2.detach(), counts, iou)
        both = torch.stack([iou, iou.transpose(1, 2)]).contiguous()
        cols = torch.empty(2 * PB, K, dtype=torch.int32, device=dev)
        nat.lsap_maximize_wrapper(2 * PB, K, both, cols)
    return _MatchedDistance.apply(mask1, mask2, cols[:PB], cols[PB:], int(loss_norm))


FUSED_GN_BACKWARD_MAX_WIDTH = 64
FUSED_GN_BACKWARD = True
ACT16_MOMENT_WIDTH = int(__import__("os").environ.get("OGC_ACT16_MOMENT_WIDTH", "64"))


def _moment_width(t):
    return ACT16_MOMENT_WIDTH if t.dtype is torch.bfloat16 else FUSED_GN_BACKWARD_MAX_WIDTH


def _pool_moment_cout(t):
    return ACT16_MOMENT_WIDTH if t.dtype is torch.bfloat16 else max(FUSED_GN_BACKWARD_MAX_WIDTH, SPARSE_POOL_MAX_COUT)


def _norm_act_conv_forward(y_prev, stats_prev, gn_weight, gn_bias, conv_weight, gn_groups, eps, relu, next_groups, pool,
                           next_gamma):
    nat = _api._native
    B, cin = y_prev.shape[0], y_prev.shape[1]
    cout = conv_weight.shape[0]
    hw = y_prev.numel() // (B * cin)
    dev = y_prev.device
    mean = torch.empty(B * gn_groups, dtype=torch.float32, device=dev)
    rstd = torch.empty_like(mean)
    a = torch.empty(B * cin, dtype=torch.float32, device=dev)
    bb = torch.empty_like(a)
    gamma, beta = gn_weight.contiguous(), gn_bias.contiguous()
    if stats_prev is not None:
        nat.group_norm_coeffs_wrapper(B, cin, hw, gn_groups, eps, None, gamma, beta, stats_prev,
                                      stats_prev.numel() // (2 * B * gn_groups), None, mean, rstd, a, bb)
    else:
        ws = nat.group_norm_ws(B, cin, gn_groups, False, dev)
        nat.group_norm_coeffs_wrapper(B, cin, hw, gn_groups, eps, y_prev, gamma, beta, None, 0, ws, mean, rstd, a, bb)
    y = torch.empty((B, cout) + tuple(y_prev.shape[2:]), dtype=y_prev.dtype, device=dev)
    w = conv_weight.contiguous()
    stats = extremes = None
    if (next_groups > 0 and next_groups <= 32 and cout % next_groups == 0 and (cout // next_groups) % 4 == 0
            and (cin <= 100 or _stats_ok(nat, B, cout, cin, hw, True))):
        stats = zeroed_empty(nat.conv1x1_gn_slots() * B * next_groups * 2, torch.float64, dev)
        if (pool and next_gamma is not None and (cin <= 100 or POOL_EXTREMES_WIDE)
                and getattr(nat, "conv1x1_gemm_affine_pool_wrapper", None) is not None):
            centres = hw // pool
            yext = torch.empty(B, cout, centres, dtype=torch.float32, device=dev)
            aext = torch.empty(B, cout, centres, dtype=torch.int32, device=dev)
            nat.conv1x1_gemm_affine_pool_wrapper(B, cout, cin, hw, relu, next_groups, pool, w, y_prev, a, bb,
                                                 next_gamma.contiguous(), y, stats, yext, aext)
            extremes = (yext, aext)
        else:
            nat.conv1x1_gemm_affine_wrapper(B, cout, cin, hw, relu, next_groups, w, y_prev, a, bb, y, stats)
    else:
        nat.conv1x1_gemm_affine_wrapper(B, cout, cin, hw, relu, 0, w, y_prev, a, bb, y, None)
    return y, stats, extremes, mean, rstd, a, bb


class _NormActConv(Function):

    @staticmethod
    def forward(ctx, y_prev, stats_prev, gn_weight, gn_bias, conv_weight, gn_groups, eps, relu, next_groups, pool=0,
                next_gamma=None):
        ctx.set_materialize_grads(False)
        y_prev = y_prev.contiguous()
        y, stats, extremes, mean, rstd, a, bb = _norm_act_conv_forward(y_prev, stats_prev, gn_weight, gn_bias, conv_weight,
                                                                       gn_groups, eps, relu, next_groups, pool, next_gamma)
        hw = y_prev.numel() // (y_prev.shape[0] * y_prev.shape[1])
        ctx.save_for_backward(y_prev, gn_weight, gn_bias, conv_weight, mean, rstd, a, bb)
        ctx.cfg = (gn_groups, relu, hw)
        if extremes is not None:
            ctx.mark_non_differentiable(stats, *extremes)
            return (y, stats) + extremes
        if stats is not None:
            ctx.mark_non_differentiable(stats)
        return y, stats

    @staticmethod
    def backward(ctx, grad_y, _grad_stats=None, *_grad_extremes):
        if grad_y is None:
            return (None,) * 11
        nat = _api._native
        y_prev, gn_weight, gn_bias, conv_weight, mean, rstd, a, bb = ctx.saved_tensors
        gn_groups, relu, hw = ctx.cfg
        B, cin = y_prev.shape[0], y_prev.shape[1]
        cout = conv_weight.shape[0]
        grad_y = grad_y.contiguous()
        w = conv_weight.contiguous()
        grad_w = zeroed_empty((cout, cin), torch.float32, y_prev.device)
        if (FUSED_GN_BACKWARD and getattr(nat, "conv1x1_dgrad_adjoint_wrapper", None) is not None and hw % 64 == 0
                and cout <= _moment_width(y_prev) and cin <= _moment_width(y_prev) and gn_groups <= 32
                and cin % gn_groups == 0):
            dev = y_prev.device
            moments = zeroed_empty((B, 2, cout, cin), torch.float32, dev)
            nat.conv1x1_wgrad_moments_wrapper(B, cin, cout, hw, relu, y_prev, a, bb, grad_y, moments)
            coef = torch.empty(B, cin, 3, dtype=torch.float32, device=dev)
            ggb = zeroed_empty((2, cin), torch.float32, dev)
            gw, gb = ggb[0], ggb[1]
            nat.gn_moments_combine_wrapper(B, cin, cout, hw, gn_groups, moments, w.view(cout, cin), a, bb, mean, rstd,
                                           gn_weight.contiguous(), grad_w, coef, gw, gb)
            grad_prev = torch.empty_like(y_prev)
            nat.conv1x1_dgrad_adjoint_wrapper(B, cin, cout, hw, relu, w.view(cout, cin), grad_y, y_prev, a, bb, coef, grad_prev)
            return grad_prev, None, gw, gb, grad_w.view_as(conv_weight), None, None, None, None, None, None
        nat.conv1x1_wgrad_affine_wrapper(B, cin, cout, hw, relu, y_prev, a, bb, grad_y, grad_w)
        if y_prev.dtype is torch.bfloat16 or (_gemm_ok(cout, hw) and _plain_gemm_mine(cout, (B, cin, hw))):
            grad_z = torch.empty_like(y_prev)
            nat.conv1x1_gemm_wrapper(B, cin, cout, hw, 1, w, grad_y, grad_z)
        else:
            grad_z = _product(w.view(cout, cin), grad_y.reshape(B, cout, hw), True).view_as(y_prev)
        grad_prev = torch.empty_like(y_prev)
        gw, gb = torch.empty_like(gn_weight), torch.empty_like(gn_bias)
        ws = nat.group_norm_ws(B, cin, gn_groups, True, y_prev.device)
        nat.group_norm_bwd_wrapper(B, cin, hw, gn_groups, relu, y_prev, gn_weight.contiguous(),
                                   gn_bias.contiguous(), mean, rstd, grad_z, grad_prev, gw, gb, ws)
        return grad_prev, None, gw, gb, grad_w.view_as(conv_weight), None, None, None, None, None, None


@_gate
def norm_act_conv_available(y_prev, gn, conv):
    if deterministic():
        return False
    if not (y_prev.is_cuda and _is_act(y_prev) and gn.affine and conv.bias is None and conv.groups == 1
            and all(k == 1 for k in conv.kernel_size) and all(v == 1 for v in conv.stride)
            and all(v == 0 for v in conv.padding)
            and getattr(_api._native, "conv1x1_gemm_affine_wrapper", None) is not None):
        return False
    hw = y_prev.numel() // max(y_prev.shape[0] * y_prev.shape[1], 1)
    if y_prev.dtype is torch.bfloat16 and _api._native.get_matmul_precision() != "bf16":
        return False
    return _gemm_ok(y_prev.shape[1], hw)


def act16_middle_ok(y_prev, gn, conv):
    return norm_act_conv_available(y_prev, gn, conv) and conv.weight.shape[0] <= 160


def norm_act_conv(y_prev, stats_prev, gn, relu, conv, next_gn=None, pool=0):
    next_groups = next_gn.num_groups if (next_gn is not None and next_gn.affine) else 0
    res = _NormActConv.apply(y_prev, stats_prev, gn.weight, gn.bias, conv.weight, gn.num_groups, gn.eps, bool(relu),
                             next_groups, int(pool) if (pool in (16, 32, 64) and next_groups) else 0,
                             next_gn.weight if next_groups else None)
    if pool:
        return res[0], res[1], (tuple(res[2:]) if len(res) > 2 else None)
    return res[0], res[1]


FIRST_PAIR_FUSED = True
FIRST_PAIR_MAX_C0 = 8

SKIP_REPEAT_STEPS = True


def live_steps(idx):
    nat = _api._native
    if not (SKIP_REPEAT_STEPS and torch.is_grad_enabled() and idx is not None and idx.is_cuda and idx.dim() == 3
            and idx.shape[2] in (32, 64) and idx.shape[1] <= 32768 and not deterministic() and getattr(nat, "live_steps_wrapper", None) is not None
            and nat.get_matmul_precision() == "fp32"):
        return None
    return nat.live_steps_wrapper((idx if idx.dtype is torch.int32 else idx.int()).contiguous())


class LiveLink:
    __slots__ = ("live", "n_live", "pair", "tail")

    def __init__(self, live):
        self.live, self.n_live = live
        self.pair = self.tail = False

    def fits(self, B, P, S):
        return (SKIP_REPEAT_STEPS and S in (32, 64) and tuple(self.live.shape) == (B, P * S // 16)
                and tuple(self.n_live.shape) == (B,) and not deterministic()
                and getattr(_api._native, "conv1x1_dgrad_adjoint_first_live_wrapper", None) is not None)


class _FirstPairConv(Function):

    @staticmethod
    def forward(ctx, x0, w1, gn_weight, gn_bias, w2, gn_groups, eps, relu, next_groups, link=None):
        ctx.set_materialize_grads(False)
        ctx.link = None
        if link is not None and x0.dim() == 4 and link.fits(x0.shape[0], x0.shape[2], x0.shape[3]):
            ctx.link, link.pair = link, True
        nat = _api._native
        B, c0 = x0.shape[0], x0.shape[1]
        c1, c2 = w1.shape[0], w2.shape[0]
        hw = x0.numel() // (B * c0)
        dev = x0.device
        slots = nat.conv1x1_gn_slots()
        w1c, w2c = w1.contiguous(), w2.contiguous()
        stats1 = zeroed_empty(slots * B * gn_groups * 2, torch.float64, dev)
        nat.first_conv_stats_wrapper(B, c1, c0, hw, gn_groups, x0, w1c, stats1)
        mean = torch.empty(B * gn_groups, dtype=torch.float32, device=dev)
        rstd = torch.empty_like(mean)
        a = torch.empty(B * c1, dtype=torch.float32, device=dev)
        bb = torch.empty_like(a)
        nat.group_norm_coeffs_wrapper(B, c1, hw, gn_groups, eps, None, gn_weight.contiguous(), gn_bias.contiguous(), stats1,
                                      slots, None, mean, rstd, a, bb)
        y2 = torch.empty((B, c2) + tuple(x0.shape[2:]), dtype=torch.float32, device=dev)
        stats2 = zeroed_empty(slots * B * next_groups * 2, torch.float64, dev)
        nat.conv1x1_gemm_affine_first_wrapper(B, c2, c1, hw, relu, next_groups, c0, w2c, x0, w1c, a, bb, y2, stats2)
        ctx.save_for_backward(x0, w1, gn_weight, w2, mean, rstd, a, bb)
        ctx.cfg = (gn_groups, relu, hw)
        ctx.mark_non_differentiable(stats2)
        return y2, stats2

    @staticmethod
    def backward(ctx, grad_y, _grad_stats=None):
        if grad_y is None:
            return (None,) * 10
        nat = _api._native
        link = ctx.link if (ctx.link is not None and ctx.link.tail) else None
        x0, w1, gn_weight, w2, mean, rstd, a, bb = ctx.saved_tensors
        gn_groups, relu, hw = ctx.cfg
        B, c0 = x0.shape[0], x0.shape[1]
        c1, c2 = w1.shape[0], w2.shape[0]
        dev = x0.device
        grad_y = grad_y.contiguous()
        w1c, w2c = w1.contiguous().view(c1, c0), w2.contiguous().view(c2, c1)
        moments = zeroed_empty((B, 2, c2, c1), torch.float32, dev)
        if link is not None:
            nat.conv1x1_wgrad_moments_first_live_wrapper(B, c1, c2, hw, relu, c0, x0.shape[3], x0, w1c, a, bb, grad_y, link.live,
                                                         link.n_live, moments)
        else:
            nat.conv1x1_wgrad_moments_first_wrapper(B, c1, c2, hw, relu, c0, x0, w1c, a, bb, grad_y, moments)
        grad_w2 = zeroed_empty((c2, c1), torch.float32, dev)
        coef = torch.empty(B, c1, 3, dtype=torch.float32, device=dev)
        ggb = zeroed_empty((2, c1), torch.float32, dev)
        nat.gn_moments_combine_wrapper(B, c1, c2, hw, gn_groups, moments, w2c, a, bb, mean, rstd, gn_weight.contiguous(),
                                       grad_w2, coef, ggb[0], ggb[1])
        grad_w1 = zeroed_empty((c1, c0), torch.float32, dev)
        if link is not None:
            nat.conv1x1_dgrad_adjoint_first_live_wrapper(B, c1, c2, hw, relu, c0, x0.shape[3], w2c, grad_y, x0, w1c, a, bb, coef,
                                                         link.live, link.n_live, grad_w1)
        else:
            nat.conv1x1_dgrad_adjoint_first_wrapper(B, c1, c2, hw, relu, c0, w2c, grad_y, x0, w1c, a, bb, coef, grad_w1)
        return None, grad_w1.view_as(w1), ggb[0], ggb[1], grad_w2.view_as(w2), None, None, None, None, None


def _plain_conv(conv):
    return (conv.bias is None and conv.groups == 1 and all(k == 1 for k in conv.kernel_size)
            and all(v == 1 for v in conv.stride) and all(v == 0 for v in conv.padding))


def first_pair_available(x, conv, gn, conv2, gn2):
    if not FIRST_PAIR_FUSED or deterministic():
        return False
    nat = _api._native
    if (getattr(nat, "conv1x1_dgrad_adjoint_first_wrapper", None) is None or not FUSED_GN_BACKWARD
            or nat.get_matmul_precision() != "fp32"):
        return False
    if not (x is not None and x.is_cuda and x.dtype == torch.float32 and x.is_contiguous() and x.dim() >= 3
            and not x.requires_grad and 1 <= x.shape[1] <= FIRST_PAIR_MAX_C0 and x.shape[0] >= 1):
        return False
    if not (_plain_conv(conv) and _plain_conv(conv2) and gn.affine and gn2.affine):
        return False
    c0, c1, c2 = x.shape[1], conv.weight.shape[0], conv2.weight.shape[0]
    hw = x.numel() // (x.shape[0] * c0)
    g1, g2 = gn.num_groups, gn2.num_groups
    return (conv.weight.shape[1] == c0 and conv2.weight.shape[1] == c1 and hw % 64 == 0
            and c1 <= FUSED_GN_BACKWARD_MAX_WIDTH and c2 <= FUSED_GN_BACKWARD_MAX_WIDTH
            and g1 <= 32 and c1 % g1 == 0 and (c1 // g1) % 4 == 0 and g2 <= 32 and c2 % g2 == 0 and (c2 // g2) % 4 == 0
            and max(c1, c2) * hw < 2 ** 31 and x.shape[0] <= 32768)


def first_pair_conv(x, conv, gn, relu, conv2, gn2, link=None):
    return _FirstPairConv.apply(x, conv.weight, gn.weight, gn.bias, conv2.weight, gn.num_groups, gn.eps, bool(relu),
                                gn2.num_groups, link)


SPARSE_POOL_BACKWARD = True
SPARSE_POOL_MAX_COUT = 64
WIDE_POOL_BACKWARD = _os.environ.get("OGC_WIDE_POOL", "1") != "0"

class _NormActConvPool(Function):

    @staticmethod
    def forward(ctx, y_prev, stats_prev, gn_weight, gn_bias, conv_weight, gn_groups, eps, relu, gn2_weight, gn2_bias,
                groups2, eps2, relu2, link=None):
        nat = _api._native
        y_prev = y_prev.contiguous()
        B, cin, P, S = y_prev.shape
        cout = conv_weight.shape[0]
        ctx.link = None
        if (link is not None and link.pair and y_prev.dtype is torch.float32 and link.fits(B, P, S)
                and cin <= _moment_width(y_prev) and cout <= _pool_moment_cout(y_prev)):
            ctx.link, link.tail = link, True
        y, stats, extremes, mean, rstd, a, bb = _norm_act_conv_forward(y_prev, stats_prev, gn_weight, gn_bias, conv_weight,
                                                                       gn_groups, eps, relu, groups2, S, gn2_weight)
        dev = y_prev.device
        out = torch.empty(B, cout, P, dtype=torch.float32, device=dev)
        arg = torch.empty(B, cout, P, dtype=torch.int32, device=dev)
        mean2 = torch.empty(B * groups2, dtype=torch.float32, device=dev)
        rstd2 = torch.empty_like(mean2)
        g2, b2 = gn2_weight.contiguous(), gn2_bias.contiguous()
        nat.group_norm_pool_extremes_wrapper(B, cout, P, S, groups2, eps2, relu2, extremes[0], extremes[1], g2, b2, out, arg,
                                             mean2, rstd2, stats, stats.numel() // (2 * B * groups2))
        ctx.save_for_backward(y_prev, gn_weight, gn_bias, conv_weight, mean, rstd, a, bb, y, gn2_weight, mean2, rstd2, out, arg,
                              extremes[0])
        ctx.cfg = (gn_groups, relu, groups2, relu2)
        return out

    @staticmethod
    def backward(ctx, grad_out):
        nat = _api._native
        (y_prev, gn_weight, gn_bias, conv_weight, mean, rstd, a, bb, y, gn2_weight, mean2, rstd2, out, arg,
         yext) = ctx.saved_tensors
        gn_groups, relu, groups2, relu2 = ctx.cfg
        B, cin, P, S = y_prev.shape
        cout, hw, dev = conv_weight.shape[0], P * S, y_prev.device
        coef2 = torch.empty(B, cout, 2, dtype=torch.float32, device=dev)
        inj = torch.empty(B, cout, P, 2, dtype=torch.float32, device=dev)
        gw2, gb2 = torch.empty_like(gn2_weight), torch.empty_like(gn2_weight)
        ws = nat.group_norm_ws(B, cout, groups2, True, dev)
        nat.group_norm_maxpool_bwd_sparse_wrapper(B, cout, P, S, groups2, relu2, y, gn2_weight.contiguous(), mean2,
                                                  rstd2, out, arg, grad_out.contiguous(), coef2, inj, gw2, gb2, ws,
                                                  yext if POOL_SUMS_FROM_EXTREMES else None)
        w = conv_weight.contiguous().view(cout, cin)
        if cin > _moment_width(y_prev) or cout > _pool_moment_cout(y_prev):
            grad_w = zeroed_empty((cout, cin), torch.float32, dev)
            nat.conv1x1_wgrad_affine_pooled_wrapper(B, cin, cout, hw, relu, S, y_prev, a, bb, y, coef2, inj, grad_w)
            grad_z = torch.empty_like(y_prev)
            nat.conv1x1_dgrad_pooled_wrapper(B, cin, cout, hw, S, w, y, coef2, inj, grad_z)
            grad_prev = torch.empty_like(y_prev)
            gw, gb = torch.empty_like(gn_weight), torch.empty_like(gn_bias)
            ws = nat.group_norm_ws(B, cin, gn_groups, True, dev)
            nat.group_norm_bwd_wrapper(B, cin, hw, gn_groups, relu, y_prev, gn_weight.contiguous(), gn_bias.contiguous(), mean,
                                       rstd, grad_z, grad_prev, gw, gb, ws)
            return (grad_prev, None, gw, gb, grad_w.view_as(conv_weight), None, None, None, gw2, gb2, None, None, None, None)
        link = ctx.link
        moments = zeroed_empty((B, 2, cout, cin), torch.float32, dev)
        if link is not None:
            nat.conv1x1_wgrad_moments_pooled_live_wrapper(B, cin, cout, hw, relu, S, y_prev, a, bb, y, coef2, inj, link.live,
                                                          link.n_live, moments)
        else:
            nat.conv1x1_wgrad_moments_pooled_wrapper(B, cin, cout, hw, relu, S, y_prev, a, bb, y, coef2, inj, moments)
        coef = torch.empty(B, cin, 3, dtype=torch.float32, device=dev)
        ggb = zeroed_empty((2, cin), torch.float32, dev)
        gw, gb = ggb[0], ggb[1]
        grad_w = torch.empty(cout, cin, dtype=torch.float32, device=dev)
        nat.gn_moments_combine_wrapper(B, cin, cout, hw, gn_groups, moments, w, a, bb, mean, rstd,
                                       gn_weight.contiguous(), grad_w, coef, gw, gb)
        grad_prev = torch.empty_like(y_prev)
        if link is not None:
            nat.conv1x1_dgrad_adjoint_pooled_live_wrapper(B, cin, cout, hw, relu, S, w, y, coef2, inj, y_prev, a, bb, coef,
                                                          link.live, link.n_live, grad_prev)
        else:
            nat.conv1x1_dgrad_adjoint_pooled_wrapper(B, cin, cout, hw, relu, S, w, y, coef2, inj, y_prev, a, bb, coef, grad_prev)
        return (grad_prev, None, gw, gb, grad_w.view_as(conv_weight), None, None, None, gw2, gb2, None, None, None, None)


@_gate
def norm_act_conv_pool_available(y_prev, gn, conv, next_gn):
    nat = _api._native
    if not (SPARSE_POOL_BACKWARD and FUSED_GN_BACKWARD and y_prev.dim() == 4 and y_prev.shape[-1] in (16, 32, 64)
            and next_gn is not None and next_gn.affine and norm_act_conv_available(y_prev, gn, conv)
            and getattr(nat, "conv1x1_dgrad_adjoint_pooled_wrapper", None) is not None
            and getattr(nat, "conv1x1_gemm_affine_pool_wrapper", None) is not None):
        return False
    cin, cout, g, g2 = y_prev.shape[1], conv.weight.shape[0], gn.num_groups, next_gn.num_groups
    if cin > _moment_width(y_prev) or cout > _pool_moment_cout(y_prev):
        B, hw = y_prev.shape[0], y_prev.shape[2] * y_prev.shape[3]
        return (WIDE_POOL_BACKWARD and getattr(nat, "conv1x1_dgrad_pooled_wrapper", None) is not None
                and hw % 64 == 0 and B * (hw // 64) >= 1024 and B <= 65535
                and g <= 32 and cin % g == 0 and g2 <= 32 and cout % g2 == 0 and (cout // g2) % 4 == 0
                and (cin <= 100 or (POOL_EXTREMES_WIDE and _stats_ok(nat, B, cout, cin, hw, True))))
    kq = (cout + 3) // 4
    lds = (64 * 4 * (kq | 1) + 320) * 4 + 4 * cout * (64 // y_prev.shape[-1]) * 16
    return (lds <= 65536 and (y_prev.shape[2] * y_prev.shape[3]) % 64 == 0 and cin <= _moment_width(y_prev)
            and cout <= _pool_moment_cout(y_prev) and g <= 32 and cin % g == 0
            and g2 <= 32 and cout % g2 == 0 and (cout // g2) % 4 == 0)

# ... 316 lines not shown
```

ogc_amd/pointnet2_cuda.py:

```python
import torch

from . import _lib


def _check(t, dtype, name):
    try:
        if t.is_cuda and t.dtype is dtype and t.is_contiguous():
            return t.data_ptr()
    except AttributeError:
        pass
    if not isinstance(t, torch.Tensor):
        raise TypeError("%s must be a torch.Tensor" % name)
    if t.device.type != "cuda":
        raise RuntimeError("%s must be a CUDA tensor (HIP device); ogc_amd has no CPU path" % name)
    if not t.is_contiguous():
        raise RuntimeError("%s must be contiguous" % name)
    if t.dtype != dtype:
        raise RuntimeError("%s must be %s, got %s" % (name, dtype, t.dtype))
    return t.data_ptr()


def _f(t, name):
    return _check(t, torch.float32, name)

# ... 633 lines not shown
         _f(coef, "coef"), op)


def first_conv_stats_wrapper(b, c1, c0, hw, groups, x0, w1, stats):
    _run("ogc_first_conv_stats", x0, b, c1, c0, hw, groups, _f(x0, "x0"), _f(w1, "w1"), _check(stats, torch.float64, "stats"))


def conv1x1_gemm_affine_first_wrapper(b, M, K, hw, relu, groups, c0, w, x0, w1, pa, pb, out, stats):
    _run("ogc_conv1x1_gemm_affine_first", x0, b, M, K, hw, int(relu), groups, c0, _f(w, "w"), _f(x0, "x0"), _f(w1, "w1"),
         _f(pa, "pa"), _f(pb, "pb"), _f(out, "out"), _check(stats, torch.float64, "stats"))


def conv1x1_wgrad_moments_first_wrapper(b, cin, cout, hw, relu, c0, x0, w1, pa, pb, grad_y, moments):
    _run("ogc_conv1x1_wgrad_moments_first", x0, b, cin, cout, hw, int(relu), c0, _f(x0, "x0"), _f(w1, "w1"), _f(pa, "pa"),
         _f(pb, "pb"), _f(grad_y, "grad_y"), _f(moments, "moments"))


def conv1x1_dgrad_adjoint_first_wrapper(b, cin, cout, hw, relu, c0, w, grad_y, x0, w1, pa, pb, coef, grad_w1):
    _run("ogc_conv1x1_dgrad_adjoint_first", x0, b, cin, cout, hw, int(relu), c0, _f(w, "w"), _f(grad_y, "grad_y"), _f(x0, "x0"),
         _f(w1, "w1"), _f(pa, "pa"), _f(pb, "pb"), _f(coef, "coef"), _f(grad_w1, "grad_w1"))


def group_norm_maxpool_bwd_sparse_wrapper(b, c, p, s, groups, relu, x, gamma, mean, rstd, out, argmax, grad_out, coef2, inj,
                                          grad_gamma, grad_beta, ws, x_at_argmax=None):
    h, (xp,) = _acts((x,), ("x",))
    _run("ogc_group_norm_maxpool_bwd_sparse" + h, x, b, c, p, s, groups, int(relu), xp,
         _opt(x_at_argmax, torch.float32, "x_at_argmax"), _f(gamma, "gamma"),
         _f(mean, "mean"), _f(rstd, "rstd"), _f(out, "out"), _i(argmax, "argmax"), _f(grad_out, "grad_out"),
         _f(coef2, "coef2"), _f(inj, "inj"), _f(grad_gamma, "grad_gamma"), _f(grad_beta, "grad_beta"),
         _check(ws, torch.float64, "ws"))


def conv1x1_wgrad_moments_pooled_wrapper(b, cin, cout, hw, relu, nsample, y_prev, pa, pb, y, coef2, inj, moments):
    h, (ypp, yp) = _acts((y_prev, y), ("y_prev", "y"))
    _run("ogc_conv1x1_wgrad_moments_pooled" + h, y_prev, b, cin, cout, hw, int(relu), nsample, ypp, _f(pa, "pa"),
         _f(pb, "pb"), yp, _f(coef2, "coef2"), _f(inj, "inj"), _f(moments, "moments"))


def conv1x1_dgrad_adjoint_pooled_wrapper(b, cin, cout, hw, relu, nsample, w, y, coef2, inj, y_prev, pa, pb, coef, grad_prev):
    h, (yp, ypp, op) = _acts((y, y_prev, grad_prev), ("y", "y_prev", "grad_prev"))
    _run("ogc_conv1x1_dgrad_adjoint_pooled" + h, y, b, cin, cout, hw, int(relu), nsample, _f(w, "w"), yp,
         _f(coef2, "coef2"), _f(inj, "inj"), ypp, _f(pa, "pa"), _f(pb, "pb"), _f(coef, "coef"), op)


def live_steps_wrapper(idx):
    B, P, S = idx.shape
    live = torch.empty(B, P * max(S // 16, 1), dtype=torch.int32, device=idx.device)
    n_live = torch.empty(B, dtype=torch.int32, device=idx.device)
    _run("ogc_live_steps", idx, B, P, S, _i(idx, "idx"), _i(live, "live"), _i(n_live, "n_live"))
    return live, n_live


def _live_args(live, n_live):
    return (_opt(live, torch.int32, "live"), _opt(n_live, torch.int32, "n_live"),
            0 if live is None else live.numel() // max(live.shape[0], 1))


def conv1x1_wgrad_moments_pooled_live_wrapper(b, cin, cout, hw, relu, nsample, y_prev, pa, pb, y, coef2, inj, live, n_live,
                                              moments):
    _run("ogc_conv1x1_wgrad_moments_pooled_live", y_prev, b, cin, cout, hw, int(relu), nsample, _f(y_prev, "y_prev"),
         _f(pa, "pa"), _f(pb, "pb"), _f(y, "y"), _f(coef2, "coef2"), _f(inj, "inj"), *_live_args(live, n_live),
         _f(moments, "moments"))


def conv1x1_dgrad_adjoint_pooled_live_wrapper(b, cin, cout, hw, relu, nsample, w, y, coef2, inj, y_prev, pa, pb, coef, live,
                                              n_live, grad_prev):
    _run("ogc_conv1x1_dgrad_adjoint_pooled_live", y, b, cin, cout, hw, int(relu), nsample, _f(w, "w"), _f(y, "y"),
         _f(coef2, "coef2"), _f(inj, "inj"), _f(y_prev, "y_prev"), _f(pa, "pa"), _f(pb, "pb"), _f(coef, "coef"),
         *_live_args(live, n_live), _f(grad_prev, "grad_prev"))


def conv1x1_wgrad_moments_first_live_wrapper(b, cin, cout, hw, relu, c0, nsample, x0, w1, pa, pb, grad_y, live, n_live, moments):
    _run("ogc_conv1x1_wgrad_moments_first_live", x0, b, cin, cout, hw, int(relu), c0, nsample, _f(x0, "x0"), _f(w1, "w1"),
         _f(pa, "pa"), _f(pb, "pb"), _f(grad_y, "grad_y"), *_live_args(live, n_live), _f(moments, "moments"))


def conv1x1_dgrad_adjoint_first_live_wrapper(b, cin, cout, hw, relu, c0, nsample, w, grad_y, x0, w1, pa, pb, coef, live, n_live,
                                             grad_w1):
    _run("ogc_conv1x1_dgrad_adjoint_first_live", x0, b, cin, cout, hw, int(relu), c0, nsample, _f(w, "w"), _f(grad_y, "grad_y"),
         _f(x0, "x0"), _f(w1, "w1"), _f(pa, "pa"), _f(pb, "pb"), _f(coef, "coef"), *_live_args(live, n_live),
         _f(grad_w1, "grad_w1"))


def mlp_chain_pool_supported(c0, c1, c2, c3, nsample):
    return bool(_lib.load().ogc_mlp_chain_pool_supported(c0, c1, c2, c3, nsample))


def mlp_chain_pool_wrapper(x, wts, biases, out):
    B, c0, P, S = x.shape
    c = [w.shape[1] for w in wts] + [0]
    _run("ogc_mlp_chain_pool", x, B, c0, c[0], c[1], c[2] if len(wts) > 2 else 0, P, S, _f(x, "x"),
         _f(wts[0], "wt1"), _f(biases[0], "b1"), _f(wts[1], "wt2"), _f(biases[1], "b2"),
         _f(wts[2], "wt3") if len(wts) > 2 else None, _f(biases[2], "b3") if len(wts) > 2 else None, _f(out, "out"))


def corr_layer_pool_supported(cf, c1, c2, c3, nsample):
    return bool(_lib.load().ogc_corr_layer_pool_supported(cf, c1, c2, c3, nsample))


def corr_layer_pool_wrapper(pos1, pos2, feat1, feat2, idx, wts, biases, out):
    B, cf, n1 = feat1.shape
    _run("ogc_corr_layer_pool", feat1, B, cf, wts[0].shape[1], wts[1].shape[1], wts[2].shape[1], n1, feat2.shape[2],
         idx.shape[2], _f(pos1, "pos1"), _f(pos2, "pos2"), _f(feat1, "feat1"), _f(feat2, "feat2"), _i(idx, "idx"),
         _f(wts[0], "wt1"), _f(biases[0], "b1"), _f(wts[1], "wt2"), _f(biases[1], "b2"), _f(wts[2], "wt3"),
         _f(biases[2], "b3"), _f(out, "out"))


def small_linear_fwd_wrapper(x, weight, bias, y):
    rows, n_in = x.shape
    _run("ogc_small_linear_fwd", x, rows, n_in, weight.shape[0], _f(x, "x"), _f(weight, "weight"),
         None if bias is None else _f(bias, "bias"), _f(y, "y"))


def small_linear_bwd_wrapper(x, weight, grad_y, grad_x, grad_weight, grad_bias):
    rows, n_in = x.shape
    _run("ogc_small_linear_bwd", x, rows, n_in, weight.shape[0], _f(x, "x"), _f(weight, "weight"), _f(grad_y, "grad_y"),
         None if grad_x is None else _f(grad_x, "grad_x"), None if grad_weight is None else _f(grad_weight, "grad_weight"),
         None if grad_bias is None else _f(grad_bias, "grad_bias"))


def slot_masks_fwd_wrapper(temperature, feats, slots, mask):
    b, d, n = feats.shape
    _run("ogc_slot_masks_fwd", feats, b, d, n, slots.shape[2], float(temperature), _f(feats, "feats"),
         _f(slots, "slots"), _f(mask, "mask"))


def slot_masks_bwd_wrapper(temperature, feats, slots, mask, grad_mask, grad_feats, grad_slots):
    b, d, n = feats.shape
    k = slots.shape[2]
    ws = torch.empty(max(int(_lib.load().ogc_slot_masks_ws_floats(b, d, n, k)), 1), dtype=torch.float32,
                     device=feats.device)
    _run("ogc_slot_masks_bwd", feats, b, d, n, k, float(temperature), _f(feats, "feats"), _f(slots, "slots"),
         _f(mask, "mask"), _f(grad_mask, "grad_mask"), _f(grad_feats, "grad_feats"), _f(grad_slots, "grad_slots"),
         _f(ws, "ws"))


def group_norm_ws(b, c, groups, backward, device):
    L = _lib.load()
    n = 2 * b * c * L.ogc_group_norm_bwd_slots() if backward else 2 * b * groups * L.ogc_group_norm_stats_slots()
    return torch.empty(max(n, 1), dtype=torch.float64, device=device)


_precision = "fp32"


def set_matmul_precision(mode):
    global _precision
    if mode not in ("fp32", "bf16"):
        raise ValueError("matmul precision must be 'fp32' or 'bf16'")
    previous = "bf16" if _lib.load().ogc_set_matmul_precision(1 if mode == "bf16" else 0) else "fp32"
    _precision = mode
    return previous


def get_matmul_precision():
    return _precision


def conv1x1_gemm_stream_supported(b, m, k, hw):
    return bool(_lib.load().ogc_conv1x1_gemm_stream_supported(int(b), int(m), int(k), int(hw)))


def conv1x1_gemm_stats_supported(b, m, k, hw, affine):
    return bool(_lib.load().ogc_conv1x1_gemm_stats_supported(int(b), int(m), int(k), int(hw), 1 if affine else 0))


# ... 42 lines not shown
```

ogc_amd/utils/nn_util.py:

```python
import numpy as np
import torch
import torch.nn as nn


class GroupNorm(nn.Sequential):

    def __init__(self, in_size, num_groups, name=""):
        super().__init__()
        gn = nn.GroupNorm(num_groups, in_size)
        nn.init.ones_(gn.weight)
        nn.init.zeros_(gn.bias)
        self.add_module(name + "gn", gn)


class _BatchNormNd(nn.Sequential):
    _cls = None

    def __init__(self, in_size, name=""):
        super().__init__()
        bn = self._cls(in_size)
        nn.init.ones_(bn.weight)
        nn.init.zeros_(bn.bias)
        self.add_module(name + "bn", bn)

# ... 75 lines not shown


class Conv1d(_ConvNd):
    _conv, _dim = nn.Conv1d, 1

    def __init__(self, in_size, out_size, kernel_size=1, stride=1, padding=0, dilation=1,
                 activation=nn.ReLU(inplace=True), bn=None, init=nn.init.kaiming_normal_, bias=True,
                 preact=False, name=""):
        super().__init__(in_size, out_size, kernel_size, stride, padding, dilation, activation, bn, init, bias,
                         preact, name)


class Conv2d(_ConvNd):
    _conv, _dim = nn.Conv2d, 2

    def __init__(self, in_size, out_size, kernel_size=(1, 1), stride=(1, 1), padding=(0, 0), dilation=(1, 1),
                 activation=nn.ReLU(inplace=True), bn=None, init=nn.init.kaiming_normal_, bias=True,
                 preact=False, name=""):
        super().__init__(in_size, out_size, kernel_size, stride, padding, dilation, activation, bn, init, bias,
                         preact, name)


class FC(nn.Sequential):

    def __init__(self, in_size, out_size, activation=nn.ReLU(inplace=True), bn=None, init=None, preact=False,
                 name=""):
        super().__init__()
        fc = nn.Linear(in_size, out_size, bias=bn is None)
        if init is not None:
            init(fc.weight)
        if bn is None:
            nn.init.zeros_(fc.bias)
        norm = None
        if bn is not None:
            norm = get_norm_layer(bn, 1, in_size=in_size if preact else out_size)
        _assemble(self, name, "fc", fc, norm, activation, preact)


class SharedMLP(nn.Sequential):

    def __init__(self, args, bn=None, activation=nn.ReLU(inplace=True), preact=False, first=False, name=""):
        super().__init__()
        for i, (c_in, c_out) in enumerate(zip(args[:-1], args[1:])):
            bare = first and preact and i == 0
            self.add_module(name + "layer%d" % i,
                            Conv2d(c_in, c_out, bn=None if bare else bn, activation=None if bare else activation,
                                   preact=preact))


def _shared_mlp_run(self, x, pool, first=None, live=None):
    from ..fused import (act16_middle_ok, group_norm_act, group_norm_act_maxpool, norm_act_conv, norm_act_conv_available,
                         norm_act_conv_pool, norm_act_conv_pool_available, pointwise_conv)
    layers = list(self.children())
    link = None
    pending = None

    def flush(p, last):
        y, stats, gn, relu, extremes = p
        if y.dtype is torch.bfloat16:
            from ..fused import act16_leave
            y, extremes = act16_leave(y), None
        if last and pool:
            return group_norm_act_maxpool(y, gn, relu, stats, extremes)
        return group_norm_act(y, gn, relu, stats)

    def block(layer):
        conv_name, norm_name, relu = layer._names
        return getattr(layer, conv_name), getattr(layer, norm_name)[0], relu

    skip = False
    for li, layer in enumerate(layers):
        if skip:
            skip = False
            continue
        fusable = isinstance(layer, _ConvNd) and layer._gn_fuse
        if (fusable and li == 0 and first is None and len(layers) >= 2 + (1 if pool else 0)
                and isinstance(layers[1], _ConvNd) and layers[1]._gn_fuse):
            from ..fused import first_pair_available, first_pair_conv
            (conv, gn, relu), (conv2, gn2, relu2) = block(layer), block(layers[1])
            if first_pair_available(x, conv, gn, conv2, gn2):
                if live is not None and pool and len(layers) == 3:
                    from ..fused import LiveLink
                    link = LiveLink(live)
                y, stats = first_pair_conv(x, conv, gn, relu, conv2, gn2, link)
                pending, skip = (y, stats, gn2, relu2, None), True
                continue
        if not fusable:
            if pending is not None:
                x, pending = flush(pending, False), None
            x = layer(x)
            continue
        conv_name, norm_name, relu = layer._names
        conv, gn = getattr(layer, conv_name), getattr(layer, norm_name)[0]
        extremes = None
        if pending is not None and pending[0].dtype is torch.bfloat16:
            tail = pool and li == len(layers) - 1
            ok = (norm_act_conv_pool_available(pending[0], pending[2], conv, gn) if tail else
                  (act16_middle_ok(pending[0], pending[2], conv) and li < len(layers) - 1))
            if not ok:
                from ..fused import act16_leave
                pending = (act16_leave(pending[0]),) + tuple(pending[1:4]) + (None,)
        if pending is not None and norm_act_conv_available(pending[0], pending[2], conv):
            if pool and li == len(layers) - 1 and pending[0].dim() == 4 and pending[0].shape[-1] in (16, 32, 64):
                if norm_act_conv_pool_available(pending[0], pending[2], conv, gn):
                    return norm_act_conv_pool(pending[0], pending[1], pending[2], pending[3], conv, gn, relu,
                                              link if li == 2 else None)
                y, stats, extremes = norm_act_conv(pending[0], pending[1], pending[2], pending[3], conv, gn,
                                                   pool=pending[0].shape[-1])
            else:
                y, stats = norm_act_conv(pending[0], pending[1], pending[2], pending[3], conv, gn)
        else:
            if pending is not None:
                x, pending = flush(pending, False), None
            y, stats = first(conv, gn) if (first is not None and li == 0) else pointwise_conv(x, conv, gn)
        pending = (y, stats, gn, relu, extremes)
    if pending is not None:
        return flush(pending, True)
    return x.max(dim=-1)[0] if pool else x


def _shared_mlp_forward(self, x):
    return _shared_mlp_run(self, x, False)


def _shared_mlp_forward_maxpool(self, x, first=None, live=None):
    return _shared_mlp_run(self, x, True, first, live)


def _shared_mlp_first_layer(self):
    layers = list(self.children())
    if not layers or not (isinstance(layers[0], _ConvNd) and layers[0]._gn_fuse):
        return None
    conv_name, norm_name, _ = layers[0]._names
    return getattr(layers[0], conv_name), getattr(layers[0], norm_name)[0]


SharedMLP.forward = _shared_mlp_forward
SharedMLP.forward_maxpool = _shared_mlp_forward_maxpool
SharedMLP.first_layer = _shared_mlp_first_layer


def knead_leading_dims(n_dim: int, data: torch.Tensor):
    if data is None:
        return None
    shape = list(data.size())
    return data.view(int(np.prod(shape[:n_dim])), *shape[n_dim:])


def break_leading_dim(dim_size: list, data: torch.Tensor):
    if data is None:
        return None
    return data.view(*dim_size, *list(data.size())[1:])


class Seq(nn.Sequential):

    def __init__(self, input_channels):
        super().__init__()
        self.count = 0
        self.current_channels = input_channels

    def _push(self, module, out_channels=None):
        self.add_module(str(self.count), module)
        self.count += 1
        if out_channels is not None:
            self.current_channels = out_channels
        return self

    def conv1d(self, out_size, kernel_size=1, stride=1, padding=0, dilation=1, activation=nn.ReLU(inplace=True),
               leaky=False, bn=None, init=nn.init.kaiming_normal_, bias=True, preact=False, name=""):
        if leaky:
            activation = nn.LeakyReLU(0.1, inplace=True)
        return self._push(Conv1d(self.current_channels, out_size, kernel_size=kernel_size, stride=stride,
                                 padding=padding, dilation=dilation, activation=activation, bn=bn, init=init,
                                 bias=bias, preact=preact, name=name), out_size)

    def conv2d(self, out_size, kernel_size=(1, 1), stride=(1, 1), padding=(0, 0), dilation=(1, 1),
               activation=nn.ReLU(inplace=True), bn=None, init=nn.init.kaiming_normal_, bias=True, preact=False,
               name=""):
        return self._push(Conv2d(self.current_channels, out_size, kernel_size=kernel_size, stride=stride,
                                 padding=padding, dilation=dilation, activation=activation, bn=bn, init=init,
                                 bias=bias, preact=preact, name=name), out_size)

    def fc(self, out_size, activation=nn.ReLU(inplace=True), bn=None, init=None, preact=False, name=""):
        return self._push(FC(self.current_channels, out_size, activation=activation, bn=bn, init=init,
                             preact=preact, name=name), out_size)

    def dropout(self, p=0.5):
        return self._push(nn.Dropout(p=p))

    def maxpool2d(self, kernel_size, stride=None, padding=0, dilation=1, return_indices=False, ceil_mode=False):
        return self._push(nn.MaxPool2d(kernel_size=kernel_size, stride=stride, padding=padding, dilation=dilation,
                                       return_indices=return_indices, ceil_mode=ceil_mode))
```

Baseline: 1777 point-clouds/s.

## Run first set-abstraction forward convolutions only over live (non-repeated) neighbour steps

After: 1840 point-clouds/s, median of 6. 1.04x the previous value.

```diff
diff --git a/include/ogc_ops.h b/include/ogc_ops.h
--- a/include/ogc_ops.h
+++ b/include/ogc_ops.h
@@ -256,6 +256,15 @@
                                          const float *grad_y, const float *x0, const float *w1, const float *pa, const float *pb,
                                          const float *coef, const int *live, const int *n_live, int live_cap, float *grad_w1,
                                          ogc_stream_t stream);
+
+int ogc_live_steps_fwd(int b, int p, int nsample, const int *idx, int *live, int *n_live, int *fwd, int *n_fwd, ogc_stream_t stream);
+int ogc_conv1x1_gemm_affine_first_live(int b, int M, int K, int hw, int relu, int groups, int c0, int nsample, const float *w,
+                                       const float *x0, const float *w1, const float *pa, const float *pb, const int *live,
+                                       const int *n_live, int live_cap, float *out, double *stats, ogc_stream_t stream);
+int ogc_conv1x1_gemm_affine_pool_live(int b, int M, int K, int hw, int relu, int groups, int nsample, const float *w,
+                                      const float *in, const float *pa, const float *pb, const float *next_gamma, const int *live,
+                                      const int *n_live, int live_cap, float *out, double *stats, float *yext, int *aext,
+                                      ogc_stream_t stream);
 
 int ogc_mlp_chain_pool_supported(int c0, int c1, int c2, int c3, int nsample);
 int ogc_mlp_chain_pool(int b, int c0, int c1, int c2, int c3, int p, int nsample, const float *x, const float *wt1,
diff --git a/ogc_amd/_lib.py b/ogc_amd/_lib.py
--- a/ogc_amd/_lib.py
+++ b/ogc_amd/_lib.py
@@ -124,6 +124,11 @@
                                              _vp],
     "ogc_conv1x1_dgrad_adjoint_first_live": [_int, _int, _int, _int, _int, _int, _int, _vp, _vp, _vp, _vp, _vp, _vp, _vp, _vp, _vp,
                                              _int, _vp, _vp],
+    "ogc_live_steps_fwd": [_int, _int, _int, _vp, _vp, _vp, _vp, _vp, _vp],
+    "ogc_conv1x1_gemm_affine_first_live": [_int, _int, _int, _int, _int, _int, _int, _int, _vp, _vp, _vp, _vp, _vp, _vp, _vp, _int,
+                                           _vp, _vp, _vp],
+    "ogc_conv1x1_gemm_affine_pool_live": [_int, _int, _int, _int, _int, _int, _int, _vp, _vp, _vp, _vp, _vp, _vp, _vp, _int, _vp,
+                                          _vp, _vp, _vp, _vp],
     "ogc_mlp_chain_pool_supported": [_int, _int, _int, _int, _int],
     "ogc_mlp_chain_pool":[_int, _int, _int, _int, _int, _int, _int, _vp, _vp, _vp, _vp, _vp, _vp, _vp, _vp, _vp],
     "ogc_corr_layer_pool_supported": [_int, _int, _int, _int, _int],
diff --git a/ogc_amd/csrc/build.py b/ogc_amd/csrc/build.py
--- a/ogc_amd/csrc/build.py
+++ b/ogc_amd/csrc/build.py
@@ -5,7 +5,7 @@
 
 HERE = os.path.dirname(os.path.abspath(__file__))
 SOURCES = ["api.hip", "det.hip", "knn.hip", "ball_query.hip", "fps.hip", "gather_group.hip", "interpolate.hip", "kabsch.hip", "rigid_icp.hip", "ground_plane.hip", "seg_eval.hip", "flow_eval.hip", "sup_loss.hip", "small_solvers.hip", "neighbour_loss.hip", "soft_nn.hip", "soft_carry.hip", "scan_prepare.hip", "kittisf_prepare.hip", "seg_loss.hip", "group_norm.hip", "batch_norm.hip", "grid.hip", "grid_ball_query.hip", "grid_knn.hip", "conv1x1.hip", "conv1x1_h.hip", "conv1x1_wgrad.hip", "attention.hip", "slot_masks.hip", "small_linear.hip", "loss_glue.hip", "mlp_chain.hip", "gn_fused_bwd.hip", "adam.hip", "gemm_chunk.hip", "chamfer.hip", "flow_step.hip"]
-HEADERS = ["ogc_common.h", "grid.h", "grid_dev.h", "conv_stage.h", "conv1x1_shared.h", "act_io.h", "norm_dev.h", "conv1x1_epilogue.h", "first_conv.h", "wgrad_tile_body.inc", "wgrad_shared_body.inc", "svd3.h", "png_unfilter.h", os.path.join("..", "..", "include", "ogc_ops.h")]
+HEADERS = ["ogc_common.h", "grid.h", "grid_dev.h", "conv_stage.h", "conv1x1_shared.h", "act_io.h", "norm_dev.h", "conv1x1_epilogue.h", "first_conv.h", "live_steps.h", "wgrad_tile_body.inc", "wgrad_shared_body.inc", "svd3.h", "png_unfilter.h", os.path.join("..", "..", "include", "ogc_ops.h")]
 LIB = os.path.join(HERE, "libogc_ops.so")
 FMAD_SOURCES = ["knn.hip", "ball_query.hip", "fps.hip", "grid.hip", "grid_ball_query.hip", "grid_knn.hip"]
 LIB_FMAD = os.path.join(HERE, "libogc_ops_fmad.so")
diff --git a/ogc_amd/csrc/conv1x1.hip b/ogc_amd/csrc/conv1x1.hip
--- a/ogc_amd/csrc/conv1x1.hip
+++ b/ogc_amd/csrc/conv1x1.hip
@@ -10,7 +10,7 @@
 
 
 template <bool TRANSPOSE_A, int KQ, bool STATS, bool PRO, bool BF, bool POOL = false, typename IT = float, typename OT = float,
-          int FIRST = 0>
+          int FIRST = 0, bool LIST = false>
 __global__ __launch_bounds__(WG_WAVES *OGC_WAVE) void conv1x1_gemm_kernel(int M, int K, int hw, int groups,
                                                                           const float *__restrict__ w,
                                                                           const IT *__restrict__ in,
@@ -18,17 +18,33 @@
                                                                           double *__restrict__ stats,
                                                                           const float *__restrict__ pa,
                                                                           const float *__restrict__ pb, int pro_relu,
-                                                                          PoolOut pool = PoolOut(), FirstIn first = FirstIn()) {
+                                                                          PoolOut pool = PoolOut(), FirstIn first = FirstIn(),
+                                                                          LiveIn ls = LiveIn()) {
     extern __shared__ __attribute__((aligned(16))) float a_lds[];
     __shared__ __attribute__((aligned(16))) float s_w1[FIRST ? FC_MAX_ROWS * FC_MAX_C0 : 4];
     __shared__ double s_stats[STATS ? 64 : 1];
     __shared__ __attribute__((aligned(16))) float s_sign[POOL ? 64 : 4];
+    __shared__ __attribute__((aligned(16))) float s_live[LIST ? WG_WAVES * LIVE_WAVE_FLOATS : 4];
     const int lane = threadIdx.x & 63, wave = threadIdx.x >> 6;
     const int j = lane & 15, kk = lane >> 4;
     const int b = blockIdx.y;
     const int p0 = (blockIdx.x * WG_WAVES + wave) * 64;
     const int Kq = (K + 3) >> 2, a_ld = ogc_a_ld(Kq);
-    const bool live = p0 < hw;
+    bool live = p0 < hw;
+    int pos = p0 + 4 * j;
+    bool lane_live = live;
+    LiveTile lt = LiveTile();
+    if constexpr (LIST) {
+        static_assert(STATS && PRO && !BF && !TRANSPOSE_A && sizeof(IT) == 4 && sizeof(OT) == 4 && (POOL || FIRST > 0),
+                      "list form: fp32, first-layer or pooled, with statistics");
+        const int n_lv = min(ls.n[b], ls.cap);
+        if ((int)blockIdx.x * 4 * WG_WAVES >= n_lv) return;
+        const int tile = blockIdx.x * WG_WAVES + wave;
+        live = 4 * tile < n_lv;
+        lt = ogc_live_tile(ls.steps + (size_t)b * ls.cap, n_lv, tile, hw, POOL && pool.s == 32 ? 5 : 6, j);
+        pos = lt.pos;
+        lane_live = live && lt.ok;
+    }
     const IT *inb = in + (size_t)b * K * hw;
     OT *outb = out + (size_t)b * M * hw;
     if (STATS && threadIdx.x < 2 * groups) s_stats[threadIdx.x] = 0.0;
@@ -38,8 +54,8 @@
         static_assert(KQ * 4 <= FC_MAX_ROWS && sizeof(IT) == 4 && !TRANSPOSE_A, "first-layer form: fp32, at most 64 rows of W1");
         ogc_first_stage_w1<WG_WAVES * OGC_WAVE>(s_w1, first.w1, K, first.c0);
         float4 x0v[FIRST];
-        ogc_first_load_raw<FIRST>(x0v, first.x0 + (size_t)b * first.c0 * hw + (live ? p0 + 4 * j : 0), first.c0, hw);
-        ogc_first_mask<FIRST>(x0v, first.c0, live);
+        ogc_first_load_raw<FIRST>(x0v, first.x0 + (size_t)b * first.c0 * hw + (lane_live ? pos : 0), first.c0, hw);
+        ogc_first_mask<FIRST>(x0v, first.c0, lane_live);
         __syncthreads();
 #pragma unroll
         for (int q = 0; q < KQ; ++q) {
@@ -51,7 +67,7 @@
 #pragma unroll
     for (int q = 0; q < KQ; ++q) {
         const int row = q * 4 + kk;
-        xin[q] = (live && q < Kq && row < K) ? ogc_ld4(inb + (size_t)row * hw + p0 + 4 * j) : make_float4(0.f, 0.f, 0.f, 0.f);
+        xin[q] = (lane_live && q < Kq && row < K) ? ogc_ld4(inb + (size_t)row * hw + pos) : make_float4(0.f, 0.f, 0.f, 0.f);
     }
     }
     if (PRO) {
@@ -205,12 +221,17 @@
 #pragma unroll
                 for (int r = 0; r < 4; ++r) {
                     const int m = m0 + a * 16 + kk * 4 + r;
-                    if (m < M) {
+                    if (m < M && (!LIST || lane_live)) {
                         const float4 o = make_float4(acc[a][0][r], acc[a][1][r], acc[a][2][r], acc[a][3][r]);
-                        ogc_st4(outb + (size_t)m * hw + p0 + 4 * j, o);
-                    }
-                }
-            if constexpr (POOL) {
+                        ogc_st4(outb + (size_t)m * hw + pos, o);
+                    }
+                }
+            if constexpr (POOL && LIST) {
+                const int centres = hw / pool.s;
+                const size_t o0 = ((size_t)b * M + m0 + kk * 4) * centres;
+                ogc_live_pool_epilogue(acc, nblk, lt, s_live + wave * LIVE_WAVE_FLOATS, s_sign, j, kk, m0, M, centres, pool.s,
+                                       pool.yext + o0, pool.aext + o0);
+            } else if constexpr (POOL) {
                 const int centres = hw / pool.s;
                 const int centre = (p0 + 4 * j) / pool.s;
                 const size_t o0 = ((size_t)b * M + m0 + kk * 4) * centres + centre;
@@ -218,23 +239,22 @@
                 else if (pool.s == 32) ogc_pool_extremes_epilogue<8>(acc, nblk, s_sign, j, kk, m0, M, centres, 32, pool.yext + o0, pool.aext + o0);
                 else ogc_pool_extremes_epilogue<4>(acc, nblk, s_sign, j, kk, m0, M, centres, 16, pool.yext + o0, pool.aext + o0);
             }
-            if (STATS) {
+            if constexpr (STATS && LIST) {
+                ogc_live_stats_epilogue(acc, nblk, lt, s_live + wave * LIVE_WAVE_FLOATS, j, kk, [&](int a, float sm, float sq) {
+                    const int m = m0 + a * 16 + kk * 4;
+                    if (m < M) {
+                        atomicAdd(&s_stats[2 * (m / cpg)], (double)sm);
+                        atomicAdd(&s_stats[2 * (m / cpg) + 1], (double)sq);
+                    }
+                });
+            } else if (STATS) {
 #pragma unroll
                 for (int a = 0; a < 4; ++a) {
                     if (a < nblk) {
-                        float sm = 0.f, sq = 0.f;
-#pragma unroll
-                        for (int r = 0; r < 4; ++r)
-#pragma unroll
-                            for (int c = 0; c < 4; ++c) {
-                                const float v = acc[a][c][r];
-                                sm += v;
-                                sq += v * v;
-                            }
-                        sm += ogc_dpp_f32<0xB1>(sm); sq += ogc_dpp_f32<0xB1>(sq);
-                        sm += ogc_dpp_f32<0x4E>(sm); sq += ogc_dpp_f32<0x4E>(sq);
-                        sm += ogc_dpp_f32<0x141>(sm); sq += ogc_dpp_f32<0x141>(sq);
-                        sm += ogc_dpp_f32<0x140>(sm); sq += ogc_dpp_f32<0x140>(sq);
+                        float sm, sq;
+                        ogc_stats_lane_sum(acc[a][0], acc[a][1], acc[a][2], acc[a][3], sm, sq);
+                        ogc_stats_quad_sum(sm, sq);
+                        ogc_stats_row_sum(sm, sq);
                         const int m = m0 + a * 16 + kk * 4;
                         if (j == 0 && m < M) {
                             const int g = m / cpg;
@@ -813,10 +833,11 @@
     return OGC_OK;
 }
 
-extern "C" int ogc_conv1x1_gemm_affine_first(int b, int M, int K, int hw, int relu, int groups, int c0, const float *w,
-                                             const float *x0, const float *w1, const float *pa, const float *pb, float *out,
-                                             double *stats, ogc_stream_t stream) {
-    const char *name = "ogc_conv1x1_gemm_affine_first";
+namespace {
+template <bool LIST>
+int gemm_affine_first_impl(const char *name, int b, int M, int K, int hw, int relu, int groups, int c0, const float *w,
+                           const float *x0, const float *w1, const float *pa, const float *pb, float *out, double *stats,
+                           ogc_stream_t stream, LiveIn ls = LiveIn()) {
     int rc = first_check(name, b, K, c0, hw, x0, w1);
     if (rc != OGC_OK) return rc;
     OGC_REQUIRE(M >= 1 && w && pa && pb && out && stats, "%s: bad shape or null pointer", name);
@@ -838,9 +859,9 @@
     FirstIn first;
     first.x0 = x0; first.w1 = w1; first.c0 = c0;
 #define OGC_GEMM_FIRST(KQV, CPV)                                                                                           \
-    hipLaunchKernelGGL((conv1x1_gemm_kernel<false, KQV, true, true, false, false, float, float, CPV>), grid,               \
+    hipLaunchKernelGGL((conv1x1_gemm_kernel<false, KQV, true, true, false, false, float, float, CPV, LIST>), grid,         \
                        dim3(WG_WAVES * OGC_WAVE), lds, s, M, K, hw, groups, w, (const float *)nullptr, out, stats, pa, pb, relu, \
-                       PoolOut(), first)
+                       PoolOut(), first, ls)
     if (Kq <= 8) {
         if (cp == 3) OGC_GEMM_FIRST(8, 3); else if (cp == 6) OGC_GEMM_FIRST(8, 6); else OGC_GEMM_FIRST(8, 8);
     } else {
@@ -850,3 +871,58 @@
     OGC_CHECK_LAUNCH(name);
     return OGC_OK;
 }
+}
+
+extern "C" int ogc_conv1x1_gemm_affine_first(int b, int M, int K, int hw, int relu, int groups, int c0, const float *w,
+                                             const float *x0, const float *w1, const float *pa, const float *pb, float *out,
+                                             double *stats, ogc_stream_t stream) {
+    return gemm_affine_first_impl<false>("ogc_conv1x1_gemm_affine_first", b, M, K, hw, relu, groups, c0, w, x0, w1, pa, pb, out,
+                                         stats, stream);
+}
+
+extern "C" int ogc_conv1x1_gemm_affine_first_live(int b, int M, int K, int hw, int relu, int groups, int c0, int nsample,
+                                                  const float *w, const float *x0, const float *w1, const float *pa,
+                                                  const float *pb, const int *live, const int *n_live, int live_cap, float *out,
+                                                  double *stats, ogc_stream_t stream) {
+    const char *name = "ogc_conv1x1_gemm_affine_first_live";
+    LiveIn ls;
+    const int rc = live_check(name, live, n_live, live_cap, hw, nsample, ls);
+    if (rc != OGC_OK) return rc;
+    return gemm_affine_first_impl<true>(name, b, M, K, hw, relu, groups, c0, w, x0, w1, pa, pb, out, stats, stream, ls);
+}
+
+extern "C" int ogc_conv1x1_gemm_affine_pool_live(int b, int M, int K, int hw, int relu, int groups, int nsample, const float *w,
+                                                 const float *in, const float *pa, const float *pb, const float *next_gamma,
+                                                 const int *live, const int *n_live, int live_cap, float *out, double *stats,
+                                                 float *yext, int *aext, ogc_stream_t stream) {
+    const char *name = "ogc_conv1x1_gemm_affine_pool_live";
+    LiveIn ls;
+    int rc = live_check(name, live, n_live, live_cap, hw, nsample, ls);
+    if (rc != OGC_OK) return rc;
+    rc = gemm_check(name, b, M, K, hw, w, in, out);
+    if (rc != OGC_OK) return rc;
+    OGC_REQUIRE(pa && pb && next_gamma && stats && yext && aext, "%s: null pointer", name);
+    if (groups < 1 || groups > 32 || M % groups != 0 || (M / groups) % 4 != 0 || K > 64 || g_matmul_bf16) {
+        ogc_set_error("%s: needs fp32 operands, 1 <= groups <= 32, (M / groups) %% 4 == 0 and K <= 64 (M=%d, groups=%d, K=%d)", name,
+                      M, groups, K);
+        return OGC_ERR_UNSUPPORTED;
+    }
+    if (b == 0) return OGC_OK;
+    hipStream_t s = (hipStream_t)stream;
+    if (ogc_zero_async(stats, sizeof(double) * 2 * GN_SLOTS * (size_t)b * groups, s) != hipSuccess) {
+        ogc_set_error("%s: memset failed", name);
+        return OGC_ERR_LAUNCH;
+    }
+    PoolOut pool;
+    pool.yext = yext; pool.aext = aext; pool.sign = next_gamma; pool.s = nsample;
+    const int Kq = (K + 3) / 4;
+    const size_t lds = (size_t)64 * ogc_a_ld(Kq) * sizeof(float);
+    dim3 grid(ogc_divup(hw, 64 * WG_WAVES), b);
+#define OGC_GEMM_POOL_LIVE(KQV)                                                                                            \
+    hipLaunchKernelGGL((conv1x1_gemm_kernel<false, KQV, true, true, false, true, float, float, 0, true>), grid,            \
+                       dim3(WG_WAVES * OGC_WAVE), lds, s, M, K, hw, groups, w, in, out, stats, pa, pb, relu, pool, FirstIn(), ls)
+    if (Kq <= 8) OGC_GEMM_POOL_LIVE(8); else OGC_GEMM_POOL_LIVE(16);
+#undef OGC_GEMM_POOL_LIVE
+    OGC_CHECK_LAUNCH(name);
+    return OGC_OK;
+}
diff --git a/ogc_amd/csrc/conv1x1_epilogue.h b/ogc_amd/csrc/conv1x1_epilogue.h
--- a/ogc_amd/csrc/conv1x1_epilogue.h
+++ b/ogc_amd/csrc/conv1x1_epilogue.h
@@ -1,5 +1,6 @@
 #pragma once
 #include "conv1x1_shared.h"
+#include "live_steps.h"
 
 namespace {
 
@@ -75,6 +76,164 @@
     }
 }
 
+template <typename ACC>
+__device__ __forceinline__ void ogc_stats_lane_sum(const ACC &c0, const ACC &c1, const ACC &c2, const ACC &c3, float &sm, float &sq) {
+    sm = 0.f; sq = 0.f;
+#pragma unroll
+    for (int r = 0; r < 4; ++r) {
+        const float v0 = c0[r], v1 = c1[r], v2 = c2[r], v3 = c3[r];
+        sm += v0; sq += v0 * v0;
+        sm += v1; sq += v1 * v1;
+        sm += v2; sq += v2 * v2;
+        sm += v3; sq += v3 * v3;
+    }
+}
+__device__ __forceinline__ void ogc_stats_quad_sum(float &sm, float &sq) {
+    sm += ogc_dpp_f32<0xB1>(sm); sq += ogc_dpp_f32<0xB1>(sq);
+    sm += ogc_dpp_f32<0x4E>(sm); sq += ogc_dpp_f32<0x4E>(sq);
+}
+__device__ __forceinline__ void ogc_stats_row_sum(float &sm, float &sq) {
+    sm += ogc_dpp_f32<0x141>(sm); sq += ogc_dpp_f32<0x141>(sq);
+    sm += ogc_dpp_f32<0x140>(sm); sq += ogc_dpp_f32<0x140>(sq);
+}
+
+struct LiveTile {
+    int pos;
+    bool ok;
+    bool tile_lead;
+    bool centre_lead;
+    int src[4];
+    bool dead[4];
+    bool member[4];
+};
+__device__ __forceinline__ LiveTile ogc_live_tile(const int *lv, int n_lv, int tile, int hw, int s_shift, int j) {
+    LiveTile lt;
+    int ent[4];
+#pragma unroll
+    for (int t = 0; t < 4; ++t) ent[t] = 4 * tile + t < n_lv ? lv[4 * tile + t] : LIVE_PAD;
+    const int e = j >> 2;
+    const int mine = e == 0 ? ent[0] : e == 1 ? ent[1] : e == 2 ? ent[2] : ent[3];
+    const int step = min(mine & LIVE_MASK, (hw >> 4) - 1);
+    const int t_shift = s_shift - 4;
+    lt.ok = mine >= 0;
+    lt.pos = lt.ok ? step * 16 + 4 * (j & 3) : 0;
+    lt.centre_lead = lt.ok && (step & ((1 << t_shift) - 1)) == 0;
+    lt.tile_lead = lt.ok;
+#pragma unroll
+    for (int s = 0; s < 4; ++s) { lt.src[s] = e; lt.dead[s] = (step & 3) != s; lt.member[s] = false; }
+#pragma unroll
+    for (int t = 0; t < 4; ++t) {
+        const int st = ent[t] & LIVE_MASK;
+        const bool same_tile = lt.ok && ent[t] >= 0 && (st >> 2) == (step >> 2);
+        if (t < e && same_tile) lt.tile_lead = false;
+        if (t > e && same_tile) {
+#pragma unroll
+            for (int s = 0; s < 4; ++s)
+                if ((st & 3) <= s) { lt.src[s] = t; lt.dead[s] = (st & 3) != s; }
+            lt.member[t] = (st >> t_shift) == (step >> t_shift);
+        }
+    }
+    return lt;
+}
+
+constexpr int LIVE_WAVE_FLOATS = 4 * 4 * 4 * 4 + 4 * 4 * 4 * 4 * 2;
+
+template <typename ACC, typename ADD>
+__device__ __forceinline__ void ogc_live_stats_epilogue(const ACC (&acc)[4][4], int nblk, const LiveTile &lt, float *wl, int j, int kk,
+                                                        ADD add) {
+    float4 *tab = reinterpret_cast<float4 *>(wl);
+    const int e = j >> 2;
+    __builtin_amdgcn_wave_barrier();
+#pragma unroll
+    for (int a = 0; a < 4; ++a) {
+        if (a < nblk) {
+            float sm, sq, dm, dq;
+            ogc_stats_lane_sum(acc[a][0], acc[a][1], acc[a][2], acc[a][3], sm, sq);
+            ogc_stats_quad_sum(sm, sq);
+            ogc_stats_lane_sum(acc[a][3], acc[a][3], acc[a][3], acc[a][3], dm, dq);
+            dm += dm; dq += dq;
+            dm += dm; dq += dq;
+            if ((j & 3) == 3) tab[(e * 4 + kk) * 4 + a] = make_float4(sm, sq, dm, dq);
+        }
+    }
+    __builtin_amdgcn_wave_barrier();
+    if (lt.tile_lead && (j & 3) == 0) {
+#pragma unroll
+        for (int a = 0; a < 4; ++a) {
+            if (a < nblk) {
+                float qm[4], qq[4];
+#pragma unroll
+                for (int s = 0; s < 4; ++s) {
+                    const float4 v = tab[(lt.src[s] * 4 + kk) * 4 + a];
+                    qm[s] = lt.dead[s] ? v.z : v.x;
+                    qq[s] = lt.dead[s] ? v.w : v.y;
+                }
+                add(a, (qm[0] + qm[1]) + (qm[2] + qm[3]), (qq[0] + qq[1]) + (qq[2] + qq[3]));
+            }
+        }
+    }
+}
+
+template <typename ACC>
+__device__ __forceinline__ void ogc_live_pool_epilogue(const ACC (&acc)[4][4], int nblk, const LiveTile &lt, float *wl, const float *sgn,
+                                                       int j, int kk, int m0, int M, int centres, int pool_s, float *ye, int *ae) {
+    float2 *tab = reinterpret_cast<float2 *>(wl + 4 * 4 * 4 * 4);
+    const int e = j >> 2, jj = j & 3;
+    const unsigned base = (unsigned)(lt.pos & (pool_s - 1));
+    __builtin_amdgcn_wave_barrier();
+#pragma unroll
+    for (int a = 0; a < 4; ++a) {
+        if (a < nblk) {
+            const float4 sg4 = *reinterpret_cast<const float4 *>(sgn + a * 16 + kk * 4);
+            const float sga[4] = {sg4.x, sg4.y, sg4.z, sg4.w};
+            float keep_hi = 0.f;
+            unsigned keep_idx = 64u;
+#pragma unroll
+            for (int r = 0; r < 4; ++r) {
+                const float sg = sga[r];
+                const float v0 = sg * acc[a][0][r], v1 = sg * acc[a][1][r];
+                const float v2 = sg * acc[a][2][r], v3 = sg * acc[a][3][r];
+                float hi = ogc_max3_f32(v0, v1, ogc_max2_f32(v2, v3));
+                hi = ogc_max_dpp_f32<0xB1>(hi);
+                hi = ogc_max_dpp_f32<0x4E>(hi);
+                unsigned idx = v3 == hi ? base + 3u : 64u;
+                idx = v2 == hi ? base + 2u : idx;
+                idx = v1 == hi ? base + 1u : idx;
+                idx = v0 == hi ? base : idx;
+                idx = min(idx, ogc_dpp_u32<0xB1>(idx));
+                idx = min(idx, ogc_dpp_u32<0x4E>(idx));
+                keep_hi = jj == r ? hi : keep_hi;
+                keep_idx = jj == r ? idx : keep_idx;
+            }
+            tab[((e * 4 + kk) * 4 + a) * 4 + jj] = make_float2(keep_hi, __uint_as_float(keep_idx));
+        }
+    }
+    __builtin_amdgcn_wave_barrier();
+    if (lt.centre_lead) {
+        const int centre = lt.pos / pool_s;
+#pragma unroll
+        for (int a = 0; a < 4; ++a) {
+            const int m = m0 + a * 16 + kk * 4 + jj;
+            if (a < nblk && m < M) {
+                float2 v[4];
+#pragma unroll
+                for (int t = 0; t < 4; ++t) v[t] = tab[((t * 4 + kk) * 4 + a) * 4 + jj];
+                float hi = e == 0 ? v[0].x : e == 1 ? v[1].x : e == 2 ? v[2].x : v[3].x;
+#pragma unroll
+                for (int t = 1; t < 4; ++t)
+                    if (lt.member[t]) hi = ogc_max2_f32(hi, v[t].x);
+                unsigned idx = 64u;
+#pragma unroll
+                for (int t = 0; t < 4; ++t)
+                    if ((t == e || lt.member[t]) && v[t].x == hi) idx = min(idx, __float_as_uint(v[t].y));
+                const size_t o = ((size_t)(a * 16 + jj)) * centres + centre;
+                ye[o] = sgn[a * 16 + kk * 4 + jj] * hi;
+                ae[o] = (int)(idx & (unsigned)(pool_s - 1));
+            }
+        }
+    }
+}
+
 template <auto KERNEL, typename... ARGS>
 bool ogc_persistent_launch(size_t lds, int lds_cap, int per_cu, long long ntiles, hipStream_t s, ARGS... args) {
     static bool raised = false;
diff --git a/ogc_amd/csrc/gn_fused_bwd.hip b/ogc_amd/csrc/gn_fused_bwd.hip
--- a/ogc_amd/csrc/gn_fused_bwd.hip
+++ b/ogc_amd/csrc/gn_fused_bwd.hip
@@ -1,21 +1,18 @@
 #include "conv1x1_shared.h"
 #include "act_io.h"
 #include "first_conv.h"
+#include "live_steps.h"
 
 namespace {
 
-constexpr int LIVE_SHIFT = 28;
-constexpr int LIVE_MASK = (1 << LIVE_SHIFT) - 1;
-struct LiveIn {
-    const int *steps = nullptr;
-    const int *n = nullptr;
-    int cap = 0;
-};
 
 constexpr int LIVE_MAX_P = 32768;
+template <bool FWD>
 __global__ __launch_bounds__(1024) void live_steps_kernel(int p, int s, const int *__restrict__ idx, int *__restrict__ steps,
-                                                          int *__restrict__ n_live) {
+                                                          int *__restrict__ n_live, int *__restrict__ fwd = nullptr,
+                                                          int *__restrict__ n_fwd = nullptr) {
     __shared__ int part[1024];
+    __shared__ int fmap[FWD ? 4 * 1024 : 4];
     __shared__ unsigned char cnt[LIVE_MAX_P];
     const int t = threadIdx.x, b = blockIdx.x, T = s >> 4;
     const int lane = t & 63, wave = t >> 6;
@@ -51,6 +48,58 @@
         for (int st = 0; st <= sl; ++st) out[at++] = (c * T + st) | (st == sl ? (T - 1 - sl) << LIVE_SHIFT : 0);
     }
     if (t == 1023) n_live[b] = part[1023];
+    if constexpr (FWD) {
+        const int cpg = 4 / T;
+        const int groups = p / cpg;
+        const int gper = (groups + 1023) / 1024;
+        const int g0 = min(t * gper, groups), g1 = min(g0 + gper, groups);
+        auto group_size = [&](int g) { return cpg == 1 ? (int)cnt[g] : (int)cnt[2 * g] + (int)cnt[2 * g + 1]; };
+        int len[4] = {0, 0, 0, 0};
+        for (int g = g0; g < g1; ++g) {
+            const int sz = group_size(g);
+#pragma unroll
+            for (int u = 0; u < 4; ++u) {
+                const int used = (u + len[u]) & 3;
+                len[u] += (used + sz > 4 ? 4 - used : 0) + sz;
+            }
+        }
+#pragma unroll
+        for (int u = 0; u < 4; ++u) fmap[u * 1024 + t] = len[u];
+        __syncthreads();
+        for (int off = 1; off < 1024; off <<= 1) {
+            int left[4] = {0, 0, 0, 0};
+            if (t >= off) {
+#pragma unroll
+                for (int u = 0; u < 4; ++u) left[u] = fmap[u * 1024 + t - off];
+            }
+            __syncthreads();
+            if (t >= off) {
+                int mine[4];
+#pragma unroll
+                for (int u = 0; u < 4; ++u) mine[u] = fmap[((u + left[u]) & 3) * 1024 + t];
+#pragma unroll
+                for (int u = 0; u < 4; ++u) left[u] += mine[u];
+            }
+            __syncthreads();
+            if (t >= off) {
+#pragma unroll
+                for (int u = 0; u < 4; ++u) fmap[u * 1024 + t] = left[u];
+            }
+            __syncthreads();
+        }
+        int *fo = fwd + (size_t)b * p * T;
+        int fat = t > 0 ? fmap[t - 1] : 0;
+        for (int g = g0; g < g1; ++g) {
+            const int used = fat & 3;
+            if (used + group_size(g) > 4)
+                for (int u = used; u < 4; ++u) fo[fat++] = LIVE_PAD;
+            for (int c = g * cpg; c < (g + 1) * cpg; ++c) {
+                const int sl = cnt[c] - 1;
+                for (int st = 0; st <= sl; ++st) fo[fat++] = (c * T + st) | (st == sl ? (T - 1 - sl) << LIVE_SHIFT : 0);
+            }
+        }
+        if (t == 1023) n_fwd[b] = fmap[1023];
+    }
 }
 
 template <int COB, int CIB, bool POOLED, typename AT = float, int FIRST = 0, bool LIST = false>
@@ -713,18 +762,6 @@
 namespace {
 int nsample_shift(int nsample) { return nsample == 16 ? 4 : nsample == 32 ? 5 : nsample == 64 ? 6 : -1; }
 
-int live_check(const char *name, const int *live, const int *n_live, int live_cap, int hw, int nsample, LiveIn &ls) {
-    OGC_REQUIRE(live && n_live, "%s: null live-step list", name);
-    if (nsample != 32 && nsample != 64) {
-        ogc_set_error("%s: the list form needs nsample 32 or 64 (nsample=%d)", name, nsample);
-        return OGC_ERR_UNSUPPORTED;
-    }
-    OGC_REQUIRE(hw >= 16 && hw % nsample == 0 && (hw >> 4) <= LIVE_MASK && live_cap >= (hw >> 4),
-                "%s: the live-step list holds %d entries per sample, hw=%d needs room for %d", name, live_cap, hw, hw >> 4);
-    ls.steps = live; ls.n = n_live; ls.cap = live_cap;
-    return OGC_OK;
-}
-
 template <typename AT>
 int wgrad_moments_impl(const char *name, int b, int cin, int cout, int hw, int relu, const AT *y_prev, const float *pa,
                        const float *pb, const AT *grad_y, const float *coef2, const float *inj, int s_shift,
@@ -1088,7 +1125,25 @@
         return OGC_ERR_UNSUPPORTED;
     }
     if (b == 0) return OGC_OK;
-    hipLaunchKernelGGL(live_steps_kernel, dim3(b), dim3(1024), 0, (hipStream_t)stream, p, s, idx, live, n_live);
+    hipLaunchKernelGGL(live_steps_kernel<false>, dim3(b), dim3(1024), 0, (hipStream_t)stream, p, s, idx, live, n_live);
     OGC_CHECK_LAUNCH("ogc_live_steps");
     return OGC_OK;
 }
+
+extern "C" int ogc_live_steps_fwd(int b, int p, int s, const int *idx, int *live, int *n_live, int *fwd, int *n_fwd,
+                                  ogc_stream_t stream) {
+    OGC_REQUIRE(b >= 0 && p >= 1, "ogc_live_steps_fwd: bad shape");
+    if ((s != 32 && s != 64) || (p * (long long)s) % 64 != 0) {
+        ogc_set_error("ogc_live_steps_fwd: needs nsample 32 or 64 and p * nsample %% 64 == 0 (p=%d, nsample=%d)", p, s);
+        return OGC_ERR_UNSUPPORTED;
+    }
+    OGC_REQUIRE(idx && live && n_live && fwd && n_fwd, "ogc_live_steps_fwd: null pointer");
+    if (p > LIVE_MAX_P) {
+        ogc_set_error("ogc_live_steps_fwd: p=%d centres per sample, at most %d", p, LIVE_MAX_P);
+        return OGC_ERR_UNSUPPORTED;
+    }
+    if (b == 0) return OGC_OK;
+    hipLaunchKernelGGL(live_steps_kernel<true>, dim3(b), dim3(1024), 0, (hipStream_t)stream, p, s, idx, live, n_live, fwd, n_fwd);
+    OGC_CHECK_LAUNCH("ogc_live_steps_fwd");
+    return OGC_OK;
+}
diff --git a/ogc_amd/csrc/live_steps.h b/ogc_amd/csrc/live_steps.h
--- /dev/null
+++ b/ogc_amd/csrc/live_steps.h
@@ -0,0 +1,28 @@
+#pragma once
+#include <cstdint>
+#include "ogc_common.h"
+
+namespace {
+
+constexpr int LIVE_SHIFT = 28;
+constexpr int LIVE_MASK = (1 << LIVE_SHIFT) - 1;
+constexpr int LIVE_PAD = -1;
+struct LiveIn {
+    const int *steps = nullptr;
+    const int *n = nullptr;
+    int cap = 0;
+};
+
+inline int live_check(const char *name, const int *live, const int *n_live, int live_cap, int hw, int nsample, LiveIn &ls) {
+    OGC_REQUIRE(live && n_live, "%s: null live-step list", name);
+    if (nsample != 32 && nsample != 64) {
+        ogc_set_error("%s: the list form needs nsample 32 or 64 (nsample=%d)", name, nsample);
+        return OGC_ERR_UNSUPPORTED;
+    }
+    OGC_REQUIRE(hw >= 16 && hw % nsample == 0 && (hw >> 4) <= LIVE_MASK && live_cap >= (hw >> 4),
+                "%s: the live-step list holds %d entries per sample, hw=%d needs room for %d", name, live_cap, hw, hw >> 4);
+    ls.steps = live; ls.n = n_live; ls.cap = live_cap;
+    return OGC_OK;
+}
+
+}
diff --git a/ogc_amd/fused.py b/ogc_amd/fused.py
--- a/ogc_amd/fused.py
+++ b/ogc_amd/fused.py
@@ -673,7 +673,7 @@
 
 
 def _norm_act_conv_forward(y_prev, stats_prev, gn_weight, gn_bias, conv_weight, gn_groups, eps, relu, next_groups, pool,
-                           next_gamma):
+                           next_gamma, live_link=None):
     nat = _api._native
     B, cin = y_prev.shape[0], y_prev.shape[1]
     cout = conv_weight.shape[0]
@@ -701,11 +701,20 @@
             centres = hw // pool
             yext = torch.empty(B, cout, centres, dtype=torch.float32, device=dev)
             aext = torch.empty(B, cout, centres, dtype=torch.int32, device=dev)
-            nat.conv1x1_gemm_affine_pool_wrapper(B, cout, cin, hw, relu, next_groups, pool, w, y_prev, a, bb,
-                                                 next_gamma.contiguous(), y, stats, yext, aext)
+            if live_link is not None:
+                nat.conv1x1_gemm_affine_pool_live_wrapper(B, cout, cin, hw, relu, next_groups, pool, w, y_prev, a, bb,
+                                                          next_gamma.contiguous(), live_link.fwd, live_link.n_fwd, y, stats,
+                                                          yext, aext)
+            else:
+                nat.conv1x1_gemm_affine_pool_wrapper(B, cout, cin, hw, relu, next_groups, pool, w, y_prev, a, bb,
+                                                     next_gamma.contiguous(), y, stats, yext, aext)
             extremes = (yext, aext)
+        elif live_link is not None:
+            raise _live_chain_broken("the pooled convolution does not take the extremes path")
         else:
             nat.conv1x1_gemm_affine_wrapper(B, cout, cin, hw, relu, next_groups, w, y_prev, a, bb, y, stats)
+    elif live_link is not None:
+        raise _live_chain_broken("the pooled convolution does not form statistics")
     else:
         nat.conv1x1_gemm_affine_wrapper(B, cout, cin, hw, relu, 0, w, y_prev, a, bb, y, None)
     return y, stats, extremes, mean, rstd, a, bb
@@ -804,6 +813,9 @@
 
 SKIP_REPEAT_STEPS = True
 
+LIVE_FORWARD = True
+LIVE_FORWARD_PAIR = True
+
 
 def live_steps(idx):
     nat = _api._native
@@ -811,20 +823,45 @@
             and idx.shape[2] in (32, 64) and idx.shape[1] <= 32768 and not deterministic() and getattr(nat, "live_steps_wrapper", None) is not None
             and nat.get_matmul_precision() == "fp32"):
         return None
-    return nat.live_steps_wrapper((idx if idx.dtype is torch.int32 else idx.int()).contiguous())
+    idx = (idx if idx.dtype is torch.int32 else idx.int()).contiguous()
+    if (LIVE_FORWARD and (idx.shape[1] * idx.shape[2]) % 64 == 0
+            and getattr(nat, "conv1x1_gemm_affine_pool_live_wrapper", None) is not None):
+        return nat.live_steps_fwd_wrapper(idx)
+    return nat.live_steps_wrapper(idx)
 
 
 class LiveLink:
-    __slots__ = ("live", "n_live", "pair", "tail")
+    __slots__ = ("live", "n_live", "fwd", "n_fwd", "pair", "tail", "forward", "forward_pair")
 
     def __init__(self, live):
-        self.live, self.n_live = live
-        self.pair = self.tail = False
+        self.live, self.n_live = live[0], live[1]
+        self.fwd, self.n_fwd = (live[2], live[3]) if len(live) == 4 else (None, None)
+        self.pair = self.tail = self.forward = self.forward_pair = False
+
+    def plan_forward(self, x0, conv2, gn2, conv3, gn3):
+        nat = _api._native
+        B, P, S = x0.shape[0], x0.shape[2], x0.shape[3]
+        c2, c3 = conv2.weight.shape[0], conv3.weight.shape[0]
+        y2 = x0.new_empty(1).expand(B, c2, P, S)
+        self.forward = bool(
+            LIVE_FORWARD and self.fwd is not None and torch.is_grad_enabled() and x0.dtype is torch.float32
+            and nat.get_matmul_precision() == "fp32" and self.fits(B, P, S) and tuple(self.fwd.shape) == tuple(self.live.shape)
+            and tuple(self.n_fwd.shape) == (B,) and POOL_SUMS_FROM_EXTREMES and (P * S) % 64 == 0
+            and getattr(nat, "conv1x1_gemm_affine_pool_live_wrapper", None) is not None
+            and c2 <= min(_moment_width(y2), 64) and c3 <= _pool_moment_cout(y2) and gn3.affine
+            and c3 % gn3.num_groups == 0 and (c3 // gn3.num_groups) % 4 == 0
+            and norm_act_conv_pool_available.__wrapped__(y2, gn2, conv3, gn3))
+        self.forward_pair = self.forward and LIVE_FORWARD_PAIR
 
     def fits(self, B, P, S):
         return (SKIP_REPEAT_STEPS and S in (32, 64) and tuple(self.live.shape) == (B, P * S // 16)
                 and tuple(self.n_live.shape) == (B,) and not deterministic()
                 and getattr(_api._native, "conv1x1_dgrad_adjoint_first_live_wrapper", None) is not None)
+
+
+def _live_chain_broken(what):
+    return RuntimeError("first level over live steps: %s — the chain was planned for the list forms (LiveLink.plan_forward) and "
+                        "what the forward pass wrote is valid at live positions only" % what)
 
 
 class _FirstPairConv(Function):
@@ -835,6 +872,9 @@
         ctx.link = None
         if link is not None and x0.dim() == 4 and link.fits(x0.shape[0], x0.shape[2], x0.shape[3]):
             ctx.link, link.pair = link, True
+        sparse = link is not None and link.forward_pair
+        if sparse and ctx.link is None:
+            raise _live_chain_broken("the first pair cannot take the list")
         nat = _api._native
         B, c0 = x0.shape[0], x0.shape[1]
         c1, c2 = w1.shape[0], w2.shape[0]
@@ -852,7 +892,11 @@
                                       slots, None, mean, rstd, a, bb)
         y2 = torch.empty((B, c2) + tuple(x0.shape[2:]), dtype=torch.float32, device=dev)
         stats2 = zeroed_empty(slots * B * next_groups * 2, torch.float64, dev)
-        nat.conv1x1_gemm_affine_first_wrapper(B, c2, c1, hw, relu, next_groups, c0, w2c, x0, w1c, a, bb, y2, stats2)
+        if sparse:
+            nat.conv1x1_gemm_affine_first_live_wrapper(B, c2, c1, hw, relu, next_groups, c0, x0.shape[3], w2c, x0, w1c, a, bb,
+                                                       link.fwd, link.n_fwd, y2, stats2)
+        else:
+            nat.conv1x1_gemm_affine_first_wrapper(B, c2, c1, hw, relu, next_groups, c0, w2c, x0, w1c, a, bb, y2, stats2)
         ctx.save_for_backward(x0, w1, gn_weight, w2, mean, rstd, a, bb)
         ctx.cfg = (gn_groups, relu, hw)
         ctx.mark_non_differentiable(stats2)
@@ -864,6 +908,8 @@
             return (None,) * 10
         nat = _api._native
         link = ctx.link if (ctx.link is not None and ctx.link.tail) else None
+        if link is None and ctx.link is not None and ctx.link.forward:
+            raise _live_chain_broken("the pooled tail did not take the list")
         x0, w1, gn_weight, w2, mean, rstd, a, bb = ctx.saved_tensors
         gn_groups, relu, hw = ctx.cfg
         B, c0 = x0.shape[0], x0.shape[1]
@@ -939,8 +985,12 @@
         if (link is not None and link.pair and y_prev.dtype is torch.float32 and link.fits(B, P, S)
                 and cin <= _moment_width(y_prev) and cout <= _pool_moment_cout(y_prev)):
             ctx.link, link.tail = link, True
+        sparse = link is not None and link.forward
+        if sparse and ctx.link is None:
+            raise _live_chain_broken("the pooled tail cannot take the list")
         y, stats, extremes, mean, rstd, a, bb = _norm_act_conv_forward(y_prev, stats_prev, gn_weight, gn_bias, conv_weight,
-                                                                       gn_groups, eps, relu, groups2, S, gn2_weight)
+                                                                       gn_groups, eps, relu, groups2, S, gn2_weight,
+                                                                       link if sparse else None)
         dev = y_prev.device
         out = torch.empty(B, cout, P, dtype=torch.float32, device=dev)
         arg = torch.empty(B, cout, P, dtype=torch.int32, device=dev)
diff --git a/ogc_amd/pointnet2_cuda.py b/ogc_amd/pointnet2_cuda.py
--- a/ogc_amd/pointnet2_cuda.py
+++ b/ogc_amd/pointnet2_cuda.py
@@ -739,6 +739,29 @@
          _f(grad_w1, "grad_w1"))
 
 
+def live_steps_fwd_wrapper(idx):
+    B, P, S = idx.shape
+    live = torch.empty(B, P * max(S // 16, 1), dtype=torch.int32, device=idx.device)
+    fwd = torch.empty_like(live)
+    n_live = torch.empty(B, dtype=torch.int32, device=idx.device)
+    n_fwd = torch.empty_like(n_live)
+    _run("ogc_live_steps_fwd", idx, B, P, S, _i(idx, "idx"), _i(live, "live"), _i(n_live, "n_live"), _i(fwd, "fwd"),
+         _i(n_fwd, "n_fwd"))
+    return live, n_live, fwd, n_fwd
+
+
+def conv1x1_gemm_affine_first_live_wrapper(b, M, K, hw, relu, groups, c0, nsample, w, x0, w1, pa, pb, fwd, n_fwd, out, stats):
+    _run("ogc_conv1x1_gemm_affine_first_live", x0, b, M, K, hw, int(relu), groups, c0, nsample, _f(w, "w"), _f(x0, "x0"),
+         _f(w1, "w1"), _f(pa, "pa"), _f(pb, "pb"), *_live_args(fwd, n_fwd), _f(out, "out"), _check(stats, torch.float64, "stats"))
+
+
+def conv1x1_gemm_affine_pool_live_wrapper(b, M, K, hw, relu, groups, nsample, w, x, pa, pb, next_gamma, fwd, n_fwd, out, stats,
+                                          yext, aext):
+    _run("ogc_conv1x1_gemm_affine_pool_live", x, b, M, K, hw, int(relu), groups, nsample, _f(w, "w"), _f(x, "x"), _f(pa, "pa"),
+         _f(pb, "pb"), _f(next_gamma, "next_gamma"), *_live_args(fwd, n_fwd), _f(out, "out"),
+         _check(stats, torch.float64, "stats"), _f(yext, "yext"), _i(aext, "aext"))
+
+
 def mlp_chain_pool_supported(c0, c1, c2, c3, nsample):
     return bool(_lib.load().ogc_mlp_chain_pool_supported(c0, c1, c2, c3, nsample))
 
diff --git a/ogc_amd/utils/nn_util.py b/ogc_amd/utils/nn_util.py
--- a/ogc_amd/utils/nn_util.py
+++ b/ogc_amd/utils/nn_util.py
@@ -181,6 +181,9 @@
                 if live is not None and pool and len(layers) == 3:
                     from ..fused import LiveLink
                     link = LiveLink(live)
+                    if x.dim() == 4 and isinstance(layers[2], _ConvNd) and layers[2]._gn_fuse:
+                        conv3, gn3, _ = block(layers[2])
+                        link.plan_forward(x, conv2, gn2, conv3, gn3)
                 y, stats = first_pair_conv(x, conv, gn, relu, conv2, gn2, link)
                 pending, skip = (y, stats, gn2, relu2, None), True
                 continue
@@ -204,11 +207,18 @@
                 if norm_act_conv_pool_available(pending[0], pending[2], conv, gn):
                     return norm_act_conv_pool(pending[0], pending[1], pending[2], pending[3], conv, gn, relu,
                                               link if li == 2 else None)
+            if link is not None and link.forward_pair:
+                raise RuntimeError("first level over live steps: the tail does not run as one pooled node, and the pair's output "
+                                   "is valid at live positions only")
+            if pool and li == len(layers) - 1 and pending[0].dim() == 4 and pending[0].shape[-1] in (16, 32, 64):
                 y, stats, extremes = norm_act_conv(pending[0], pending[1], pending[2], pending[3], conv, gn,
                                                    pool=pending[0].shape[-1])
             else:
                 y, stats = norm_act_conv(pending[0], pending[1], pending[2], pending[3], conv, gn)
         else:
+            if link is not None and link.forward_pair:
+                raise RuntimeError("first level over live steps: the tail cannot fold the norm into its convolution, and the "
+                                   "pair's output is valid at live positions only")
             if pending is not None:
                 x, pending = flush(pending, False), None
             y, stats = first(conv, gn) if (first is not None and li == 0) else pointwise_conv(x, conv, gn)
```
